# WilliamYi96/HGR-Net

Hardware: AMD Instinct MI355X
Metric: images/sec over 21K-class hierarchy, batch 512; hit@1 parity vs reference (higher is better)
Workload: dtype f16

## Files before the change

### hgr-net_amd/_lib.py

```python
from __future__ import annotations

import ctypes as C
import os
from pathlib import Path

import torch

_HERE = Path(__file__).resolve().parent
LIB_PATH = Path(os.environ.get("HGR_LIB", _HERE / "lib" / "libhgr.so"))

HGR_BF16, HGR_F16 = 0, 1
EPI_NONE, EPI_BIAS, EPI_BIAS_QUICKGELU, EPI_BIAS_RESIDUAL, EPI_BIAS_RELU, EPI_BIAS_ADD16_RELU, EPI_ACCUM, EPI_QGELU_GRAD16 = 0, 1, 2, 3, 4, 5, 6, 7

_p, _i, _l, _f = C.c_void_p, C.c_int, C.c_int64, C.c_float

SIGNATURES = {
    "hgr_gemm_nt": [_p, _l, _p, _l, _p, _l, _p, _p, _l, _i, _i, _i, _i, _i, _i, _p],
    "hgr_gemm_set_tile": [_i],
    "hgr_gemm_set_tail": [_i, _i],
    "hgr_gemm_set_persist": [_i],
    "hgr_gemm_set_ws": [_i],
    "hgr_gemm_set_p8": [_i],
    "hgr_im2col_patches": [_p, _p, _i, _i, _i, _i, _i, _p],
    "hgr_im2col_patches_ex": [_p, _p, _i, _i, _i, _i, _i, _i, _i, _p],
    "hgr_vit_assemble": [_p, _p, _p, _i, _i, _i, _p],
    "hgr_preprocess_bicubic": [_p, _p, _p, _p, _p, _p, _i, _p, _p, _i, _p, _p, C.POINTER(C.c_float), C.POINTER(C.c_float), _i, _i, _p],
    "hgr_im2col_patches_u8": [_p, _p, _i, _i, _i, _i, _i, _i, C.POINTER(C.c_float), C.POINTER(C.c_float), _i, _p],
    "hgr_vit_embed_ln": [_p, _p, _p, _p, _p, _p, _i, _i, _i, _f, _p],
    "hgr_layernorm": [_p, _p, _p, _p, _i, _i, _l, _p, _f, _i, _i, _p],
    "hgr_mha": [_p, _p, _i, _i, _i, _i, _i, _p],
    "hgr_mha_rows": [_p, _p, _i, _i, _i, _i, _i, _i, _p],
    "hgr_mha_stats": [_p, _p, _p, _i, _i, _i, _i, _i, _p],
    "hgr_text_embed": [_p, _l, _p, _p, _p, _i, _i, _i, _i, _p],
    "hgr_eot_index": [_p, _l, _p, _i, _i, _p],
    "hgr_l2norm_rows": [_p, _p, _p, _i, _i, _i, _p],
    "hgr_topk_rows": [_p, _l, _p, _i, _i, _p, _p, _i, _p],
    "hgr_level_argmax": [_p, _l, _p, _i, _p, _i, _p, _p, _i, _p],
    "hgr_eval_rows": [_p, _l, _i, _p, _p, _p, _i, _i, _p, _p, _p, _i, _i, _p, _p, _p, _i, _p],
    "hgr_conv3x3_nhwc": [_p, _p, _p, _p, _i, _i, _i, _i, _i, _i, _i, _i, _p],
    "hgr_conv3x3_pool2_nhwc": [_p, _p, _p, _p, _i, _i, _i, _i, _i, _i, _i, _p],
    "hgr_stem_conv1": [_p, _p, _p, _p, _i, _i, _i, _i, _i, _p],
    "hgr_stem_im2col": [_p, _p, _i, _i, _i, _p],
    "hgr_avgpool2_nhwc": [_p, _p, _i, _i, _i, _i, _i, _p],
    "hgr_attnpool_tokens": [_p, _p, _p, _i, _i, _i, _i, _p],
    "hgr_attnpool_attend": [_p, _p, _p, _p, _i, _i, _i, _i, _p],
    "hgr_transpose16": [_p, _l, _p, _l, _i, _i, _p],
    "hgr_transpose16_colsum": [_p, _l, _p, _l, _i, _i, _i, _p, _i, _f, _p, _p],
    "hgr_colsum": [_p, _l, _i, _i, _i, _i, _p, _i, _f, _p, _p],
    "hgr_cast16": [_p, _p, _l, _i, _p],
    "hgr_cast16_transpose": [_p, _l, _p, _l, _p, _l, _i, _i, _i, _p],
    "hgr_quickgelu16": [_p, _p, _p, _l, _i, _i, _p],
    "hgr_layernorm_bwd": [_p, _i, _p, _p, _p, _p, _p, _p, _i, _i, _l, _p, _f, _i, _p],
    "hgr_layernorm_bwd_cast": [_p, _i, _p, _p, _p, _p, _p, _p, _p, _i, _i, _l, _p, _f, _i, _p],
    "hgr_layernorm_bwd_cast_colsum": [_p, _i, _p, _p, _p, _p, _p, _p, _p, _p, _i, _i, _l, _p, _f, _i, _p],
    "hgr_layernorm_bwd_scratch_floats": [_i, _i],
    "hgr_mha_bwd": [_p, _p, _p, _p, _i, _i, _i, _i, _i, _p],
    "hgr_mha_bwd_stats": [_p, _p, _p, _p, _p, _i, _i, _i, _i, _i, _p],
    "hgr_mha_bwd_colsum": [_p, _p, _p, _p, _p, _p, _i, _i, _i, _i, _i, _p],
    "hgr_ce_rows": [_p, _l, _p, _i, _i, _f, _p, _p, _l, _p],
    "hgr_l2norm_bwd": [_p, _p, _p, _i, _i, _i, _p],
    "hgr_matmul_f32": [_p, _l, _l, _p, _l, _l, _p, _l, _i, _i, _i, _f, _i, _p],
    "hgr_embed_scatter_add": [_p, _l, _p, _p, _i, _i, _i, _i, _p],
    "hgr_rows_axpy": [_p, _l, _p, _p, _i, _i, _f, _p],
    "hgr_rows_gather": [_p, _p, _p, _i, _i, _p],
    "hgr_ctx_splice": [_p, _p, _p, _i, _i, _i, _i, _p],
    "hgr_ctx_splice_bwd": [_p, _p, _i, _i, _i, _i, _p],
    "hgr_sumsq": [_p, _l, _p, _p],
    "hgr_eval_counters": [_p, _i, _p, _i, _p, _p, _i, _p, _p, _i, _p, _i, _p],
    "hgr_eval_counters_rows": [_p, _i, _p, _p, _p, _i, _p, _p, _p, _i, _p, _i, _p],
    "hgr_eval_report_rows": [_p, _i, _p, _p, _p, _i, _p, _p, _p, _i, _p, _i, _p],
    "hgr_path_scores": [_p, _l, _p, _l, _i, _p, _p, _p, _i, _p],
    "hgr_subtree_hedge": [_p, _l, _i, _p, _p, _p, _f, _p, _i, _p, _p, _p, _l, _i, _p],
    "hgr_hedge_counters_rows": [_p, _i, _p, _p, _p, _i, _p, _i, _p],
    "hgr_set_ranks": [_p, _l, _i, _p, _p, _i, _p, _p, _p, _i, _p],
    "hgr_set_counters_rows": [_p, _p, _i, _p, _p, _i, _p, _p, _p, _i, _p, _i, _p],
    "hgr_dgp_score_rows": [_p, _l, _i, _i, _i, _f, _p, _i, _p, _i, _p, _p, _p, _p, _i, _i, _p],
    "hgr_dot_f32":[_p, _p, _l, _p, _f, _i, _p],
    "hgr_conv3x3_nhwc_plain": [_p, _p, _p, _i, _i, _i, _i, _i, _i, _i, _p],
    "hgr_gemm_nt_splitk": [_p, _l, _p, _l, _p, _l, _i, _i, _i, _i, _i, _p],
    "hgr_gemm_tn_splitk": [_p, _l, _p, _l, _p, _l, _i, _i, _i, _i, _i, _p],
    "hgr_gemm_tn_tile": [_i, _i],
    "hgr_gemm_plan_capture": [_p, _i],
    "hgr_conv3x3_wgrad_splitk": [_p, _l, _p, _p, _l, _i, _i, _i, _i, _i, _i, _i, _p],
    "hgr_relu_bwd16": [_p, _p, _p, _l, _i, _p],
    "hgr_add16": [_p, _p, _p, _l, _i, _p],
    "hgr_avgpool2_bwd_nhwc": [_p, _p, _i, _i, _i, _i, _i, _p],
    "hgr_attnpool_tokens_bwd": [_p, _p, _i, _i, _i, _i, _p],
    "hgr_im2col3x3_t": [_p, _p, _i, _i, _i, _i, _l, _i, _p],
    "hgr_bn_fold": [_p, _p, _p, _p, _p, _f, _p, _p, _i, _i, _i, _i, _i, _p],
    "hgr_bn_unfold_grad": [_p, _l, _p, _p, _p, _p, _p, _f, _p, _p, _p, _i, _i, _i, _p],
    "hgr_csr_group_aggregate": [_p, _l, _p, _p, _p, _p, _i, _p, _p, _p, _p, _i, _p, _p, _p, _p, _i, _p, _p, _l, _i, _f, _i, _p],
    "hgr_csr_group_att_grad": [_p, _l, _p, _p, _l, _p, _l, _p, _l, _p, _p, _p, _p, _i, _p, _p, _p, _i, _p, _p, _p, _i, _p, _p, _i, _f, _p],
    "hgr_dgp_loss_head": [_p, _l, _p, _p, _l, _i, _i, _p, _p, _p, _l, _i, _p],
    "hgr_dropout_counter": [_p, _l, _p, _l, _i, _i, _i, _i, _i, _p],
    "hgr_adam_l2": [_p, _p, _p, _p, _l, _f, _f, _f, _f, _f, _i, _p],
    "hgr_cnzsl_std_chain_fwd": [_p, _l, _p, _p, _p, _p, _p, _p, _l, _p, _l, _p, _i, _i, _i, _f, _f, _p],
    "hgr_cnzsl_std_chain_bwd": [_p, _l, _p, _l, _p, _l, _p, _p, _p, _l, _p, _i, _i, _f, _p],
    "hgr_bias_relu_f32": [_p, _l, _p, _p, _l, _i, _i, _p],
    "hgr_relu_bwd_colsum_f32": [_p, _l, _p, _l, _p, _l, _p, _p, _i, _i, _p],
    "hgr_gemm_nt_res_stats": [_p, _l, _p, _l, _p, _p, _l, _p, _p, _i, _i, _i, _i, _p],
    "hgr_vit_head": [_p, _p, _l, _l, _p, _p, _f, _p, _p, _i, _i, _i, _i, _p],
    "hgr_gemm_nt_res_stats_guard": [_p, _l, _p, _l, _p, _p, _l, _p, _p, _f, _p, _i, _i, _i, _i, _p],
    "hgr_gemm_nt_ln": [_p, _l, _p, _l, _p, _l, _p, _p, _p, _f, _i, _i, _i, _i, _i, _p],
    "hgr_gemm_nt_ln_mha": [_p, _l, _p, _l, _p, _p, _p, _f, _p, _l, _i, _i, _i, _i, _i, _p],
    "hgr_gemm_nt_bias_gelu_dual": [_p, _l, _p, _l, _p, _l, _p, _l, _p, _i, _i, _i, _i, _p],
    "hgr_gemm_nt_qgelu_grad_colsum": [_p, _l, _p, _l, _p, _l, _p, _l, _p, _i, _i, _i, _i, _p],
    "hgr_vit_embed_ln_stats": [_p, _p, _p, _p, _p, _p, _p, _p, _i, _i, _i, _f, _i, _p],
    "hgr_vit_patch_embed_ln_ok": [_i, _i, _i, _i, _i],
    "hgr_vit_patch_embed_ln": [_p, _p, _p, _p, _p, _p, _p, _p, _p, _i, _i, _i, _i, _f, _i, _p],
    "hgr_row_stats16": [_p, _p, _p, _p, _i, _i, _i, _p],
    "hgr_pair_rows_f32": [_p, _p, _p, _i, _i, _l, _p, _i, _p],
    "hgr_logits_eval_workspace_bytes": [_i, _i],
    "hgr_logits_eval": [_p, _p, _i, _i, _i, _p, _p, _p, _i, _p, _p, _i, _p, _i, _i, _p, _p, _p, _p, _i, _p],
    "hgr_logits_eval_tile_stage": [_p, _p, _i, _i, _i, _p, _p, _p, _i, _p, _p, _i, _p, _i, _i, _p, _p, _p, _p, _i, _p],
    "hgr_logits_eval_row_stage": [_p, _p, _i, _i, _i, _p, _p, _p, _i, _p, _p, _i, _p, _i, _i, _p, _p, _p, _p, _i, _p],
    "hgr_comm_unique_id": [_p],
    "hgr_comm_init": [_i, _i, _p],
    "hgr_comm_destroy": [],
    "hgr_comm_rank": [],
    "hgr_comm_world": [],
    "hgr_allreduce": [_p, _p, _l, _i, _i, _p],
    "hgr_allgather": [_p, _p, _l, _i, _p],
    "hgr_broadcast": [_p, _l, _i, _i, _p],
    "hgr_adamw": [_p, _p, _p, _p, _l, _f, _f, _f, _f, _f, _i, _p, _f, _f, _p],
}


class GemmLaunch(C.Structure):
    _fields_ = [(name, C.c_int32) for name in ("kernel", "variant", "epilogue", "out_f32", "act", "grid_x", "grid_y", "tiles_m", "tiles_n", "total",
                                                "nbig", "big_panels", "tiles_m_half", "group", "m_fastest", "vec_ok", "row0", "rows")]


class HgrError(RuntimeError):
    pass


_lib = None


ABI_VERSION = 5


def load() -> C.CDLL:
    global _lib
    if _lib is not None:
        return _lib
    if not LIB_PATH.is_file():
        raise HgrError(f"{LIB_PATH} not found: build it with `python -c 'import __graft_entry__ as g; g.build()'` "
                       f"or `make -C {_HERE / 'csrc'}`; there is no CPU fallback")
    lib = C.CDLL(str(LIB_PATH))
    lib.hgr_abi_version.restype = _i
    lib.hgr_last_error.restype = C.c_char_p
    for name, argtypes in SIGNATURES.items():
        fn = getattr(lib, name)
        fn.argtypes = argtypes
        fn.restype = _l if name.endswith(("_scratch_floats", "_workspace_bytes")) else _i
    if lib.hgr_abi_version() != ABI_VERSION:
        raise HgrError(f"libhgr.so ABI {lib.hgr_abi_version()} != {ABI_VERSION} (include/hgr.h): stale build, run `make -C {_HERE / 'csrc'}`")
    _lib = lib
    return lib


import threading

_tls = threading.local()


def set_muted(on: bool) -> bool:
    prev = getattr(_tls, "muted", False)
    _tls.muted = bool(on)
    return prev


def muted() -> bool:
    return getattr(_tls, "muted", False)


def call(name: str, *args) -> None:
    if getattr(_tls, "muted", False):
        return
    lib = load()
    rc = getattr(lib, name)(*args)
    if rc != 0:
        raise HgrError(f"{name} failed ({rc}): {lib.hgr_last_error().decode()}")
```

### hgr-net_amd/csrc/hgr_gemm.hip

```cpp
#include "hgr_gemm_common.h"

using namespace hgr_gemm;

int hgr_conv3x3_c32_launch(const void *x, const void *w, const float *bias, void *out, int B, int H, int W, int Cout, int Kp,
                           int dtype, int relu, void *stream, int pool, int C);

namespace {
constexpr int BM = 128, BN = 128;

HgrKnob<> k_group{"HGR_GEMM_GROUP", 0, [](int v) { return v < 0 ? 0 : v; }};
HgrKnob<> k_tail{"HGR_DUO_TAIL", 1}, k_pb{"HGR_DUO_PB", -1};
HgrKnob<double> k_half_cost{"HGR_DUO_HALF_COST", 0.55, [](double v) { return v > 0.1 ? v : 0.55; }};
HgrKnob<> k_tile{"HGR_GEMM_TILE", 0};
HgrKnob<> k_split{"HGR_GEMM_SPLIT", 1};
HgrKnob<> k_conv_direct{"HGR_CONV_DIRECT", 1}, k_conv_duo{"HGR_CONV_DUO", 1};
HgrKnob<> k_persist{"HGR_DUO_PERSIST", 1, hgr_knob_bool};
HgrKnob<> k_ws{"HGR_WS", 0, hgr_knob_bool};
HgrKnob<> k_p8{"HGR_P8", 2, [](int v) { return v >= 0 && v <= 2 ? v : 2; }};

int duo_group() { return k_group.get() ? k_group.get() : 4; }
int duo_group_for(int tiles_n) { return k_group.get() ? k_group.get() : (tiles_n <= 8 ? 1 : 4); }
int duo_dbg() {
    static const int d = hgr_lab_env("HGR_GEMM_DBG");
    return d;
// ... 266 lines not shown
GemmLaunch plan_conv3x3(const GemmArgs &a, int64_t in_pixels, bool relu, bool out16_aligned) {
    const int C = a.cC, Cout = a.N, Kp = a.K, stride = a.cStride, force = k_tile.get(), epi = relu ? HGR_EPI_BIAS_RELU : HGR_EPI_NONE;
    const int64_t t256 = (int64_t)((a.M + 255) / 256) * ((Cout + 255) / 256);
    const int waste256 = (Cout + 255) / 256 * 256 - Cout, waste128 = (Cout + 127) / 128 * 128 - Cout;
    const bool big = relu && force != 128 && Kp >= 128 && Cout >= 128 && (t256 >= 160 || force == 256) && waste256 <= waste128;
    const int64_t tduo = (int64_t)((a.M + 255) / 256) * ((Cout + 127) / 128);
    if (k_conv_duo.get() && relu && a.cUni && stride == 1 && Cout % 128 == 0 && Kp == 9 * C && tduo >= 256 && out16_aligned &&
        in_pixels * C * 2 < (1ll << 31) && (int64_t)Cout * Kp * 2 < (1ll << 32) && force == 0)
        return plan_duo(a, 5, HGR_EPI_BIAS_RELU, false);
    if (big) return plan_tiles(HGR_KERNEL_256, 1, HGR_EPI_BIAS_RELU, false, a.M, Cout, 256, 256);
    if (Cout <= 64 && a.M >= 1024) return plan_tiles(HGR_KERNEL_128, V128_CONV_TALL, epi, false, a.M, 1, 256, 1);
    return plan_tiles(HGR_KERNEL_128, V128_CONV, epi, false, a.M, Cout, BM, BN);
}

int conv3x3_launch(const void *x, const void *w, const float *bias, void *out,
                   int B, int H, int W, int C, int Cout, int stride, int Kp, int dtype, bool relu, void *stream) {
    CaptureScope capture;
    HGR_REQUIRE(x && w && out && (bias || !relu), "hgr_conv3x3_nhwc: null operand");
    HGR_REQUIRE(B >= 1 && H >= 1 && W >= 1 && Cout >= 1 && (stride == 1 || stride == 2), "hgr_conv3x3_nhwc: bad geometry B=%d H=%d W=%d Cout=%d stride=%d", B, H, W, Cout, stride);
    HGR_REQUIRE(C >= 8 && C % 8 == 0 && C <= 16384, "hgr_conv3x3_nhwc: C=%d must be a multiple of 8 in [8, 16384]", C);
    HGR_REQUIRE(Kp >= 9 * C && Kp % BK == 0, "hgr_conv3x3_nhwc: Kp=%d must be >= 9*C and a multiple of %d", Kp, BK);
    HGR_REQUIRE(hgr_aligned(x, 16) && hgr_aligned(w, 16) && hgr_aligned(out, 8) && (!bias || hgr_aligned(bias, 16)) && Cout % 4 == 0, "hgr_conv3x3_nhwc: misaligned operand / Cout %% 4 != 0");
    HGR_REQUIRE(dtype == HGR_BF16 || dtype == HGR_F16, "hgr_conv3x3_nhwc: bad dtype %d", dtype);
    if (const int direct = conv_direct_channels(C, Cout, stride, Kp, (int64_t)B * H * W, hgr_aligned(out, 16))) {
        if (cap_out) { *cap_out = hgr_gemm_launch{HGR_KERNEL_CONV_DIRECT, direct, relu ? HGR_EPI_BIAS_RELU : HGR_EPI_NONE, 0, relu}; return HGR_OK; }
        return hgr_conv3x3_c32_launch(x, w, bias, out, B, H, W, Cout, Kp, dtype, relu ? 1 : 0, stream, 0, direct);
    }
    const int Ho = (H + 2 - 3) / stride + 1, Wo = (W + 2 - 3) / stride + 1;
    const int64_t M64 = (int64_t)B * Ho * Wo;
    HGR_REQUIRE(M64 < (1ll << 31), "hgr_conv3x3_nhwc: too many output pixels");
    GemmArgs a = gemm_args(x, 0, w, Kp, out, Cout, (int)M64, Cout, Kp, true, 0);
    a.bias = bias; a.m_fastest = 0;
    a.cH = H; a.cW = W; a.cC = C; a.cStride = stride; a.cHo = Ho; a.cWo = Wo;
    a.cMagic = (unsigned)(((1ull << 32) + (unsigned)C - 1) / (unsigned)C);
    a.cUni = (C % 64 == 0) ? 1 : 0;
    const GemmLaunch L = plan_conv3x3(a, (int64_t)B * H * W, relu, hgr_aligned(out, 16));
    return gemm_run("hgr_conv3x3_nhwc", a, &L, 1, dtype, stream);
}
}

extern "C" int hgr_conv3x3_nhwc(const void *x, const void *w, const float *bias, void *out,
                                int B, int H, int W, int C, int Cout, int stride, int Kp, int dtype, void *stream) {
    return conv3x3_launch(x, w, bias, out, B, H, W, C, Cout, stride, Kp, dtype, true, stream);
}

extern "C" int hgr_conv3x3_nhwc_plain(const void *x, const void *w, void *out, int B, int H, int W, int C, int Cout, int Kp,
                                      int dtype, void *stream) {
    return conv3x3_launch(x, w, nullptr, out, B, H, W, C, Cout, 1, Kp, dtype, false, stream);
}

extern "C" int hgr_gemm_nt_splitk(const void *A, int64_t lda, const void *W, int64_t ldw, float *partial, int64_t ldc,
                                  int M, int N, int K, int kc, int dtype, void *stream) {
    CaptureScope capture;
    HGR_REQUIRE(A && W && partial, "hgr_gemm_nt_splitk: null operand");
    HGR_REQUIRE(M >= 1 && N >= 1 && K >= BK && K % BK == 0 && kc >= BK && kc % BK == 0, "hgr_gemm_nt_splitk: bad shape M=%d N=%d K=%d kc=%d", M, N, K, kc);
    HGR_REQUIRE(lda >= K && ldw >= K && lda % 8 == 0 && ldw % 8 == 0 && hgr_aligned(A, 16) && hgr_aligned(W, 16), "hgr_gemm_nt_splitk: operands must be 16-byte aligned with leading dimensions %% 8 == 0");
    HGR_REQUIRE(ldc >= N && ldc % 4 == 0 && hgr_aligned(partial, 16), "hgr_gemm_nt_splitk: partial must be 16-byte aligned, ldc %% 4 == 0");
    HGR_REQUIRE(dtype == HGR_BF16 || dtype == HGR_F16, "hgr_gemm_nt_splitk: bad dtype %d", dtype);
    const int S = (K + kc - 1) / kc;
    HGR_REQUIRE(S <= 65535, "hgr_gemm_nt_splitk: %d splits exceed the grid limit", S);
    GemmArgs a = gemm_args(A, lda, W, ldw, partial, ldc, M, N, K, true, 0);
    a.m_fastest = 0; a.kc = kc; a.csplit = (int64_t)M * ldc;
    const bool big = k_tile.get() != 128 && M >= 256 && N >= 256 && kc >= 128 && (K - (S - 1) * kc) >= 128;
    const GemmLaunch L = big ? plan_tiles(HGR_KERNEL_256, 0, HGR_EPI_NONE, true, M, N, 256, 256, (unsigned)S)
                             : plan_tiles(HGR_KERNEL_128, V128_PLAIN, HGR_EPI_NONE, true, M, N, BM, BN, (unsigned)S);
    return gemm_run("hgr_gemm_nt_splitk", a, &L, 1, dtype, stream);
}

namespace {
int ln_common_checks(const char *who, const void *A, int64_t lda, const void *W, int64_t ldw, int M, int N, int K, int dtype) {
    HGR_REQUIRE(A && W, "%s: null operand", who);
    HGR_REQUIRE(M >= 1 && N >= 128 && N % 128 == 0 && K >= 128 && K % 64 == 0, "%s: bad shape M=%d N=%d K=%d (N %% 128 == 0, K %% 64 == 0, K >= 128)", who, M, N, K);
    HGR_REQUIRE(lda >= K && ldw >= K && lda % 8 == 0 && ldw % 8 == 0 && hgr_aligned(A, 16) && hgr_aligned(W, 16), "%s: operands must be 16-byte aligned with leading dimensions %% 8 == 0", who);
    HGR_REQUIRE((int64_t)M * lda * 2 < (1ll << 32) && (int64_t)N * ldw * 2 < (1ll << 32) && N < (1 << 20), "%s: operands beyond 4 GB / N >= 2^20", who);
    HGR_REQUIRE(dtype == HGR_BF16 || dtype == HGR_F16, "%s: bad dtype %d", who, dtype);
    return HGR_OK;
}
}

extern "C" int hgr_gemm_nt_res_stats(const void *A, int64_t lda, const void *W, int64_t ldw, void *xh, void *xl, int64_t ldx,
                                     const float *bias, float *stats, int M, int N, int K, int dtype, void *stream) {
    return hgr_gemm_nt_res_stats_guard(A, lda, W, ldw, xh, xl, ldx, bias, stats, 0.f, nullptr, M, N, K, dtype, stream);
}

extern "C" int hgr_gemm_nt_res_stats_guard(const void *A, int64_t lda, const void *W, int64_t ldw, void *xh, void *xl, int64_t ldx,
                                           const float *bias, float *stats, float guard_sumsq, uint32_t *flag,
                                           int M, int N, int K, int dtype, void *stream) {
    CaptureScope capture;
    if (int rc = ln_common_checks("hgr_gemm_nt_res_stats", A, lda, W, ldw, M, N, K, dtype)) return rc;
    HGR_REQUIRE(!flag || (guard_sumsq > 0.f && hgr_aligned(flag, 4)), "hgr_gemm_nt_res_stats_guard: flag needs guard_sumsq > 0 and 4-byte alignment");
    HGR_REQUIRE(xh && xl && bias && stats, "hgr_gemm_nt_res_stats: null xh / xl / bias / stats");
    HGR_REQUIRE(ldx >= N && ldx % 8 == 0 && ldx < (1 << 23) && hgr_aligned(xh, 16) && hgr_aligned(xl, 16), "hgr_gemm_nt_res_stats: xh / xl must be 16-byte aligned, ldx %% 8 == 0, ldx < 2^23");
    HGR_REQUIRE(hgr_aligned(bias, 16) && hgr_aligned(stats, 8), "hgr_gemm_nt_res_stats: bias must be 16-byte, stats 8-byte aligned");
    GemmArgs a = gemm_args(A, lda, W, ldw, nullptr, 0, M, N, K, true, duo_dbg());
    a.bias = bias;
    a.ln_stats = stats; a.ln_slots = N / 64; a.ln_xh = xh; a.ln_xl = xl; a.ln_ldx = ldx;
    a.ln_flag = flag; a.ln_guard = guard_sumsq;
    const GemmLaunch L = k_ws.get() && k_tile.get() == 0 && ws_covers(M, N, K, WS_LNP) ? plan_ws(M, N, WS_LNP, HGR_EPI_BIAS_RESIDUAL, 0)
                                                                                        : plan_duo(a, 1, HGR_EPI_BIAS_RESIDUAL, true);
    return gemm_run("hgr_gemm_nt_res_stats", a, &L, 1, dtype, stream);
}

extern "C" int hgr_gemm_nt_ln(const void *X16, int64_t ldx, const void *Wfold, int64_t ldw, void *C, int64_t ldc,
                              const float *ln_s, const float *ln_c, const float *stats, float eps,
                              int M, int N, int K, int dtype, int act, void *stream) {
    CaptureScope capture;
    if (int rc = ln_common_checks("hgr_gemm_nt_ln", X16, ldx, Wfold, ldw, M, N, K, dtype)) return rc;
    HGR_REQUIRE(C && ln_s && ln_c && stats, "hgr_gemm_nt_ln: null C / ln_s / ln_c / stats");
    HGR_REQUIRE(K % 128 == 0, "hgr_gemm_nt_ln: the row width K=%d must be a multiple of 128 (two 64-column statistic slots per 16-byte load)", K);
    HGR_REQUIRE(ldc >= N && ldc % 8 == 0 && ldc < (1 << 23) && hgr_aligned(C, 16), "hgr_gemm_nt_ln: C must be 16-byte aligned with ldc %% 8 == 0, ldc < 2^23");
    HGR_REQUIRE(hgr_aligned(ln_s, 16) && hgr_aligned(ln_c, 16) && hgr_aligned(stats, 16), "hgr_gemm_nt_ln: ln_s / ln_c / stats must be 16-byte aligned");
    HGR_REQUIRE(act == 0 || act == 1, "hgr_gemm_nt_ln: act must be 0 (none) or 1 (QuickGELU), got %d", act);
    GemmArgs a = gemm_args(X16, ldx, Wfold, ldw, C, ldc, M, N, K, true, duo_dbg());
    a.ln_stats = const_cast<float *>(stats); a.ln_slots = K / 64; a.ln_eps = eps; a.ln_s = ln_s; a.ln_c = ln_c;
    const int epi = act ? HGR_EPI_BIAS_QUICKGELU : HGR_EPI_BIAS;
    const GemmLaunch L = k_tile.get() == 0 && p8_wanted(M, N, K)                           ? plan_p8(M, N, act)
                         : k_ws.get() && k_tile.get() == 0 && ws_covers(M, N, K, WS_LNC) ? plan_ws(M, N, WS_LNC, epi, act)
                                                                                          : plan_duo(a, 2, epi, false);
    return gemm_run("hgr_gemm_nt_ln", a, &L, 1, dtype, stream);
}

extern "C" int hgr_gemm_nt_bias_gelu_dual(const void *A, int64_t lda, const void *W, int64_t ldw, void *pre, int64_t ldpre, void *post, int64_t ldpost,
                                          const float *bias, int M, int N, int K, int dtype, void *stream) {
    CaptureScope capture;
    if (int rc = ln_common_checks("hgr_gemm_nt_bias_gelu_dual", A, lda, W, ldw, M, N, K, dtype)) return rc;
    HGR_REQUIRE(pre && post && bias, "hgr_gemm_nt_bias_gelu_dual: null pre / post / bias");
    HGR_REQUIRE(ldpre >= N && ldpost >= N && ldpre % 8 == 0 && ldpost % 8 == 0 && ldpre < (1 << 23) && ldpost < (1 << 23) && hgr_aligned(pre, 16) && hgr_aligned(post, 16) && hgr_aligned(bias, 16),
                "hgr_gemm_nt_bias_gelu_dual: pre / post / bias must be 16-byte aligned, leading dimensions >= N, %% 8 == 0, < 2^23");
    GemmArgs a = gemm_args(A, lda, W, ldw, pre, ldpre, M, N, K, true, duo_dbg());
    a.bias = bias; a.ln_xh = post; a.ln_ldx = ldpost;
    const GemmLaunch L = plan_duo(a, 4, HGR_EPI_BIAS, false);
    return gemm_run("hgr_gemm_nt_bias_gelu_dual", a, &L, 1, dtype, stream);
}

extern "C" int hgr_gemm_nt_qgelu_grad_colsum(const void *A, int64_t lda, const void *W, int64_t ldw, void *C, int64_t ldc, const void *pre, int64_t ldpre,
                                             float *colsum_part, int M, int N, int K, int dtype, void *stream) {
    CaptureScope capture;
    if (int rc = ln_common_checks("hgr_gemm_nt_qgelu_grad_colsum", A, lda, W, ldw, M, N, K, dtype)) return rc;
    HGR_REQUIRE(C && pre && colsum_part, "hgr_gemm_nt_qgelu_grad_colsum: null C / pre / colsum_part");
    HGR_REQUIRE(ldc >= N && ldpre >= N && ldc % 8 == 0 && ldpre % 8 == 0 && ldc < (1 << 20) && ldpre < (1 << 20) && hgr_aligned(C, 16) && hgr_aligned(pre, 16) && hgr_aligned(colsum_part, 16),
                "hgr_gemm_nt_qgelu_grad_colsum: C / pre / colsum_part must be 16-byte aligned, leading dimensions >= N, %% 8 == 0, < 2^20");
    GemmArgs a = gemm_args(A, lda, W, ldw, C, ldc, M, N, K, true, duo_dbg());
    a.res = (const float *)pre; a.ldr = ldpre;
    a.colsum = colsum_part; a.colsum_units = (M + 63) / 64;
    const GemmLaunch L = plan_duo(a, 0, HGR_EPI_QGELU_GRAD16, false);
    return gemm_run("hgr_gemm_nt_qgelu_grad_colsum", a, &L, 1, dtype, stream);
}

#define HGR_LE_PARAMS const void *feat16, const void *zsl_perm16, int rows, int D, int n_perm, const int32_t *tpos_perm, const int32_t *epos_perm, \
    const int32_t *level_first, int n_levels, const int32_t *filler_pos, const int32_t *train_cols, int n_train, const int32_t *test_cols, int n_test, int k, \
    int32_t *out_level, int32_t *out_top1, int32_t *out_topk, void *workspace, int dtype, void *stream
#define HGR_LE_ARGS feat16, zsl_perm16, rows, D, n_perm, tpos_perm, epos_perm, level_first, n_levels, filler_pos, train_cols, n_train, test_cols, n_test, k, \
    out_level, out_top1, out_topk, workspace, dtype, stream
static int logits_eval_stages(int stages, HGR_LE_PARAMS);
extern "C" int hgr_logits_eval(HGR_LE_PARAMS) { return logits_eval_stages(3, HGR_LE_ARGS); }
extern "C" int hgr_logits_eval_tile_stage(HGR_LE_PARAMS) { return logits_eval_stages(1, HGR_LE_ARGS); }
extern "C" int hgr_logits_eval_row_stage(HGR_LE_PARAMS) { return logits_eval_stages(2, HGR_LE_ARGS); }

int hgr_logits_eval_rows_launch(const void *feat, const void *zslp, int D, int S, const unsigned long long *keys, const float *tmax,
                                const int *gp1, const float *gm2, const int32_t *level_first, int n_levels, const int32_t *filler_pos, const int32_t *train_cols, int n_train,
                                const int32_t *epos, const int32_t *test_cols, int n_test, int k, int32_t *out_level, int32_t *out_top1,
                                int32_t *out_topk, int rows, int dtype, void *stream);

extern "C" int64_t hgr_logits_eval_workspace_bytes(int rows, int n_perm) {
    if (rows < 1 || n_perm < 96 || n_perm % 96) return -1;
    return (int64_t)rows * (n_perm / 32) * 32;
}

static int logits_eval_stages(int stages, const void *feat16, const void *zsl_perm16, int rows, int D, int n_perm,
                               const int32_t *tpos_perm, const int32_t *epos_perm, const int32_t *level_first,
                               int n_levels, const int32_t *filler_pos, const int32_t *train_cols, int n_train,
                               const int32_t *test_cols, int n_test, int k,
                               int32_t *out_level, int32_t *out_top1, int32_t *out_topk, void *workspace, int dtype, void *stream) {
    HGR_REQUIRE(feat16 && zsl_perm16 && tpos_perm && epos_perm && level_first && filler_pos && train_cols && out_level && workspace, "hgr_logits_eval: null operand");
    HGR_REQUIRE(rows >= 1 && D >= 128 && D % 128 == 0 && D <= 1024, "hgr_logits_eval: rows=%d D=%d unsupported (D %% 128 == 0, D <= 1024)", rows, D);
    HGR_REQUIRE(n_perm >= 96 && n_perm % 96 == 0 && n_perm / 32 <= 1024, "hgr_logits_eval: n_perm=%d must be a multiple of 96 and <= 32768 (32-column level-aligned slices, 96-column slabs)", n_perm);
    HGR_REQUIRE(n_levels >= 1 && n_levels <= 32 && n_train >= 1, "hgr_logits_eval: bad sizes (n_levels <= 32)");
    HGR_REQUIRE(k == 0 || (out_topk && test_cols && k >= 1 && k <= 32 && n_test >= k), "hgr_logits_eval: bad top-k arguments");
    HGR_REQUIRE(hgr_aligned(feat16, 16) && hgr_aligned(zsl_perm16, 16) && hgr_aligned(tpos_perm, 16) && hgr_aligned(epos_perm, 16) && hgr_aligned(workspace, 16), "hgr_logits_eval: operands must be 16-byte aligned");
    HGR_REQUIRE(dtype == HGR_BF16 || dtype == HGR_F16, "hgr_logits_eval: bad dtype %d", dtype);
    HGR_REQUIRE((int64_t)rows * D * 2 < (1ll << 32) && (int64_t)n_perm * D * 2 < (1ll << 32), "hgr_logits_eval: operands beyond 4 GB");
    const int S = n_perm / 32;
    SlabArgs a;
    a.A = (const char *)feat16; a.lda = D; a.W = (const char *)zsl_perm16; a.ldw = D; a.M = rows; a.K = D; a.Np = n_perm;
    a.tpos = tpos_perm; a.epos = epos_perm; a.S = S;
    { static const int d = hgr_lab_env("HGR_LS_DBG"); a.dbg = d; }
    a.ev_key = (unsigned long long *)workspace;
    a.ev_tmax = (float *)((char *)workspace + (size_t)rows * S * 8);
    a.ev_p1 = (int *)((char *)workspace + (size_t)rows * S * 16);
    a.ev_m2 = (float *)((char *)workspace + (size_t)rows * S * 24);
    if (stages & 1) launch_logits_slab(a, dtype, (hipStream_t)stream);
    HGR_CHECK_LAUNCH("hgr_logits_eval (tile stage)");
    if (!(stages & 2)) return HGR_OK;
    return hgr_logits_eval_rows_launch(feat16, zsl_perm16, D, S, a.ev_key, a.ev_tmax, a.ev_p1, a.ev_m2, level_first, n_levels, filler_pos, train_cols, n_train,
                                       epos_perm, test_cols, n_test, k, out_level, out_top1, out_topk, rows, dtype, stream);
}
```

### hgr-net_amd/csrc/hgr_gemm_common.h

```cpp
#pragma once
#include "hgr_common.h"
#include <stdlib.h>
#include <type_traits>

namespace hgr_gemm {

constexpr int BK = 64;

struct GemmArgs {
    const char *A = nullptr; int64_t lda = 0;
    const char *W = nullptr; int64_t ldw = 0;
    void *C = nullptr; int64_t ldc = 0;
    const float *bias = nullptr;
    const float *res = nullptr; int64_t ldr = 0;
    int M = 0, N = 0, K = 0;
    int tiles_m = 0, tiles_n = 0;
    int m_fastest = 0;
    int vec_ok = 0;
    int dbg = 0;
    int cH = 0, cW = 0, cC = 0, cStride = 0, cHo = 0, cWo = 0;
    unsigned cMagic = 0;
    int cUni = 0;
    int kc = 0; int64_t csplit = 0;
    float *ln_stats = nullptr; int ln_slots = 0; float ln_eps = 0.f;
// ... 91 lines not shown
    return o;
}

__host__ __device__ constexpr bool epi_has_bias(int epi) { return epi != HGR_EPI_NONE && epi != HGR_EPI_ACCUM && epi != HGR_EPI_QGELU_GRAD16; }
__host__ __device__ constexpr bool epi_has_idn16(int epi) { return epi == HGR_EPI_BIAS_ADD16_RELU || epi == HGR_EPI_QGELU_GRAD16; }

template <int DT, int EPI, bool OUT32>
__device__ __forceinline__ void store_quad(const GemmArgs &p, f32x4 v, int m, int n) {
    typedef typename T16<DT>::elem E;
    if (n + 3 < p.N && p.vec_ok) {
        if (epi_has_bias(EPI)) v += *(const f32x4 *)(p.bias + n);
        if (EPI == HGR_EPI_ACCUM) v += *(const f32x4 *)((const float *)p.C + (int64_t)m * p.ldc + n);
        const f32x4 v0 = v;
        f32x4 gq = (f32x4){0.f, 0.f, 0.f, 0.f};
        if (EPI == HGR_EPI_BIAS_QUICKGELU) {
#pragma unroll
            for (int e = 0; e < 4; ++e) v[e] = quick_gelu(v[e]);
        }
        if (EPI == HGR_EPI_BIAS_RESIDUAL) v += *(const f32x4 *)(p.res + (int64_t)m * p.ldr + n);
        if (epi_has_idn16(EPI)) {
            const typename T16<DT>::vec4 idn = *(const typename T16<DT>::vec4 *)((const E *)(const void *)p.res + (int64_t)m * p.ldr + n);
#pragma unroll
            for (int e = 0; e < 4; ++e) {
                if (EPI == HGR_EPI_QGELU_GRAD16) { gq[e] = quick_gelu_grad((float)idn[e]); v[e] = v[e] * gq[e]; }
                else v[e] = v[e] + (float)idn[e];
            }
        }
        if (EPI == HGR_EPI_BIAS_RELU || EPI == HGR_EPI_BIAS_ADD16_RELU) {
#pragma unroll
            for (int e = 0; e < 4; ++e) v[e] = fmaxf(v[e], 0.f);
        }
        if (OUT32) *(f32x4 *)((float *)p.C + (int64_t)m * p.ldc + n) = v;
        else if (EPI == HGR_EPI_BIAS_QUICKGELU || EPI == HGR_EPI_QGELU_GRAD16) {
            typename T16<DT>::vec4 o;
#pragma unroll
            for (int e = 0; e < 4; ++e) o[e] = EPI == HGR_EPI_BIAS_QUICKGELU ? quick_gelu16<DT>(v0[e]) : mul16<DT>(v0[e], gq[e]);
            *(typename T16<DT>::vec4 *)((E *)p.C + (int64_t)m * p.ldc + n) = o;
        } else *(typename T16<DT>::vec4 *)((E *)p.C + (int64_t)m * p.ldc + n) = cvt4<DT>(v[0], v[1], v[2], v[3]);
        return;
    }
    for (int e = 0; e < 4 && n + e < p.N; ++e) {
        float x = v[e];
        if (epi_has_bias(EPI)) x += p.bias[n + e];
        if (EPI == HGR_EPI_ACCUM) x += ((const float *)p.C)[(int64_t)m * p.ldc + n + e];
        const float x0 = x;
        float gx = 0.f;
        if (EPI == HGR_EPI_BIAS_QUICKGELU) x = quick_gelu(x);
        if (EPI == HGR_EPI_BIAS_RESIDUAL) x += p.res[(int64_t)m * p.ldr + n + e];
        if (EPI == HGR_EPI_BIAS_ADD16_RELU) x += (float)((const E *)(const void *)p.res)[(int64_t)m * p.ldr + n + e];
        if (EPI == HGR_EPI_QGELU_GRAD16) { gx = quick_gelu_grad((float)((const E *)(const void *)p.res)[(int64_t)m * p.ldr + n + e]); x *= gx; }
        if (EPI == HGR_EPI_BIAS_RELU || EPI == HGR_EPI_BIAS_ADD16_RELU) x = fmaxf(x, 0.f);
        if (OUT32) ((float *)p.C)[(int64_t)m * p.ldc + n + e] = x;
        else if (EPI == HGR_EPI_BIAS_QUICKGELU) ((E *)p.C)[(int64_t)m * p.ldc + n + e] = quick_gelu16<DT>(x0);
        else if (EPI == HGR_EPI_QGELU_GRAD16) ((E *)p.C)[(int64_t)m * p.ldc + n + e] = mul16<DT>(x0, gx);
        else ((E *)p.C)[(int64_t)m * p.ldc + n + e] = (E)x;
    }
}

template <int DT, int EPI>
__device__ __forceinline__ f32x4 load_addend(const GemmArgs &p, int m, int n) {
    typedef typename T16<DT>::elem E;
    if (EPI == HGR_EPI_ACCUM) return *(const f32x4 *)((const float *)p.C + (int64_t)m * p.ldc + n);
    if (EPI == HGR_EPI_BIAS_RESIDUAL) return *(const f32x4 *)(p.res + (int64_t)m * p.ldr + n);
    if (epi_has_idn16(EPI)) {
        const typename T16<DT>::vec4 idn = *(const typename T16<DT>::vec4 *)((const E *)(const void *)p.res + (int64_t)m * p.ldr + n);
        return (f32x4){(float)idn[0], (float)idn[1], (float)idn[2], (float)idn[3]};
    }
    return (f32x4){0.f, 0.f, 0.f, 0.f};
}

template <int DT, int EPI, bool OUT32>
__device__ __forceinline__ void store_quad_full(const GemmArgs &p, f32x4 v, f32x4 bq, f32x4 addend, int m, int n) {
    typedef typename T16<DT>::elem E;
    if (epi_has_bias(EPI)) v += bq;
    if (!OUT32 && (EPI == HGR_EPI_BIAS_QUICKGELU || EPI == HGR_EPI_QGELU_GRAD16)) {
        typename T16<DT>::vec4 o;
#pragma unroll
        for (int e = 0; e < 4; ++e) o[e] = EPI == HGR_EPI_BIAS_QUICKGELU ? quick_gelu16<DT>(v[e]) : mul16<DT>(v[e], quick_gelu_grad(addend[e]));
        *(typename T16<DT>::vec4 *)((E *)p.C + (int64_t)m * p.ldc + n) = o;
        return;
    }
    if (EPI == HGR_EPI_BIAS_QUICKGELU) {
#pragma unroll
        for (int e = 0; e < 4; ++e) v[e] = quick_gelu(v[e]);
    }
    if (EPI == HGR_EPI_ACCUM || EPI == HGR_EPI_BIAS_RESIDUAL || EPI == HGR_EPI_BIAS_ADD16_RELU) v += addend;
    if (EPI == HGR_EPI_QGELU_GRAD16) {
#pragma unroll
        for (int e = 0; e < 4; ++e) v[e] *= quick_gelu_grad(addend[e]);
    }
    if (EPI == HGR_EPI_BIAS_RELU || EPI == HGR_EPI_BIAS_ADD16_RELU) {
#pragma unroll
        for (int e = 0; e < 4; ++e) v[e] = fmaxf(v[e], 0.f);
    }
    if (OUT32) *(f32x4 *)((float *)p.C + (int64_t)m * p.ldc + n) = v;
    else *(typename T16<DT>::vec4 *)((E *)p.C + (int64_t)m * p.ldc + n) = cvt4<DT>(v[0], v[1], v[2], v[3]);
}


__device__ __forceinline__ __amdgpu_buffer_rsrc_t dma_rsrc(const void *base) {
    return __builtin_amdgcn_make_buffer_rsrc(const_cast<void *>(base), 0, (int)0xFFFFFFFFu, 0x00020000);
}
__device__ __forceinline__ void dma16(__amdgpu_buffer_rsrc_t rsrc, const char *base, unsigned voff, int soff, char *lds_dst) {
#if defined(HGR_DMA_GLOBAL) && HGR_DMA_GLOBAL
    __builtin_amdgcn_global_load_lds((const AS1 void *)(base + soff + voff), (AS3 void *)lds_dst, 16, 0, 0);
#else
    __builtin_amdgcn_raw_ptr_buffer_load_lds(rsrc, (AS3 void *)lds_dst, 16, (int)voff, soff, 0, 0);
#endif
}

#define HGR_RWAIT(N) do { __builtin_amdgcn_sched_barrier(0); \
    asm volatile("s_waitcnt vmcnt(" #N ") lgkmcnt(0)\n\ts_barrier" ::: "memory"); __builtin_amdgcn_sched_barrier(0); } while (0)
#define HGR_RBAR() do { __builtin_amdgcn_sched_barrier(0); \
    asm volatile("s_waitcnt lgkmcnt(0)\n\ts_barrier" ::: "memory"); __builtin_amdgcn_sched_barrier(0); } while (0)
#define HGR_MBAR() do { __builtin_amdgcn_sched_barrier(0); \
    asm volatile("s_barrier" ::: "memory"); __builtin_amdgcn_sched_barrier(0); } while (0)


template <int NR, int NW, int NV, int M_, int NM = 16>
__device__ __forceinline__ void mfma16_interleave_step() {
    if constexpr (M_ < NM) {
        __builtin_amdgcn_sched_group_barrier(0x008, 1, 0);
        constexpr int DR = (M_ + 1) * NR / NM - M_ * NR / NM, DW = (M_ + 1) * NW / NM - M_ * NW / NM, DV = (M_ + 1) * NV / NM - M_ * NV / NM;
        if constexpr (DR > 0) __builtin_amdgcn_sched_group_barrier(0x100, DR, 0);
        if constexpr (DW > 0) __builtin_amdgcn_sched_group_barrier(0x200, DW, 0);
        if constexpr (DV > 0) __builtin_amdgcn_sched_group_barrier(0x020, DV, 0);
        mfma16_interleave_step<NR, NW, NV, M_ + 1, NM>();
    }
}
template <int NR, int NW, int NV>
__device__ __forceinline__ void mfma16_interleave() { mfma16_interleave_step<NR, NW, NV, 0>(); }
template <int NR, int NW, int NV>
__device__ __forceinline__ void mfma8_interleave() { mfma16_interleave_step<NR, NW, NV, 0, 8>(); }

enum { V128_PLAIN = 0, V128_TALL = 1, V128_CONV = 2, V128_CONV_TALL = 3 };
void launch_128(const GemmArgs &a, int dtype, int epi, bool out32, int variant, dim3 grid, hipStream_t s);
void launch_256(const GemmArgs &a, int dtype, int epi, bool out32, bool conv, dim3 grid, hipStream_t s);
void launch_duo(const GemmArgs &a, int dtype, int epi, bool out32, int ln, dim3 grid, hipStream_t s);
enum { WS_PLAIN = 0, WS_LNC = 1, WS_LNP = 2 };
bool ws_covers(int M, int N, int K, int mode);
int ws_cus();
void launch_ws(const GemmArgs &a, int dtype, int mode, int act, bool hasb, dim3 grid, hipStream_t s);
bool p8_covers(int M, int N, int K);
void launch_p8(const GemmArgs &a, int dtype, int act, dim3 grid, hipStream_t s);

struct SlabArgs {
    const char *A = nullptr; int64_t lda = 0;
    const char *W = nullptr; int64_t ldw = 0;
    int M = 0, K = 0, Np = 0;
    const int *tpos = nullptr, *epos = nullptr;
    unsigned long long *ev_key = nullptr;
    float *ev_tmax = nullptr, *ev_m2 = nullptr; int *ev_p1 = nullptr;
    int S = 0;
    int dbg = 0;
};
void launch_logits_slab(const SlabArgs &a, int dtype, hipStream_t s);

}
```

### hgr-net_amd/csrc/hgr_logits_slab.hip

```cpp
#include "hgr_gemm_common.h"

namespace hgr_gemm {

namespace {
constexpr int LS_NT = 512;
constexpr int LS_PA0 = 0, LS_PA1 = 32768, LS_PW = 65536, LS_STAGE = 81920, LS_LDS = 2 * LS_STAGE;

template <int DT>
__global__ __launch_bounds__(LS_NT) void logits_slab(SlabArgs p) {
    typedef typename T16<DT>::vec8 vec8;
    __shared__ __attribute__((aligned(1024))) char smem[LS_LDS];

    const int tid = threadIdx.x;
    const int lane = tid & 63;
    const int wave = __builtin_amdgcn_readfirstlane(tid >> 6);
    const int pg = wave >> 2;
    const int r = lane & 15, g = lane >> 4;
    const int n0 = blockIdx.x * 96, m0 = blockIdx.y * 512;

    unsigned oA0[4], oA1[4], oW[2];
#pragma unroll
    for (int i = 0; i < 4; ++i) {
        const int id = (i * 8 + wave) * 64 + lane;
        const int pr = id >> 3, c = (id & 7) ^ (pr & 7);
        const int tr = (pr >> 5) * 64 + (pr & 31);
        oA0[i] = (unsigned)(((int64_t)min(m0 + tr, p.M - 1) * p.lda + c * 8) * 2);
        oA1[i] = (unsigned)(((int64_t)min(m0 + tr + 32, p.M - 1) * p.lda + c * 8) * 2);
        if (i < 2) oW[i] = (unsigned)(((int64_t)(n0 + min(pr, 95)) * p.ldw + c * 8) * 2);
    }
    unsigned tw[6], ta;
    {
        const int spr = p.K >> 5;
        const int nw = 96 * spr;
#pragma unroll
        for (int u = 0; u < 6; ++u) {
            const int id = min(tid + u * LS_NT, nw - 1);
            tw[u] = HGR_LAB_ON(p.dbg & 16) ? 0u : *(const unsigned *)(p.W + ((int64_t)(n0 + id / spr) * p.ldw) * 2 + (id % spr) * 64);
        }
        const int rows_here = min(512, p.M - m0), na = rows_here * spr;
        const int id = min((int)(blockIdx.x >> 3) * LS_NT + tid, na - 1);
        ta = *(const unsigned *)(p.A + ((int64_t)(m0 + id / spr) * p.lda) * 2 + (id % spr) * 64);
    }
    char *const ldsw = smem + wave * 1024;
    const __amdgpu_buffer_rsrc_t rA = dma_rsrc(p.A), rW = dma_rsrc(p.W);
    auto issueA = [&](const unsigned (&off)[4], int piece, int t) {
        if (HGR_LAB_ON(p.dbg & 2)) return;
        char *dst = ldsw + (t & 1) * LS_STAGE + piece;
#pragma unroll
        for (int i = 0; i < 4; ++i) dma16(rA, p.A, off[i], t * 128, dst + i * 8192);
    };
    auto issueW = [&](int t) {
        if (HGR_LAB_ON(p.dbg & 4)) return;
        char *dst = ldsw + (t & 1) * LS_STAGE + LS_PW;
#pragma unroll
        for (int i = 0; i < 2; ++i) dma16(rW, p.W, oW[i], t * 128, dst + i * 8192);
    };

    f32x4 acc[4][6];
#pragma unroll
    for (int i = 0; i < 4; ++i)
#pragma unroll
        for (int j = 0; j < 6; ++j) acc[i][j] = (f32x4){0.f, 0.f, 0.f, 0.f};

    const int nk = p.K / 64;
    const int offA = (wave * 32 + r) * 128;
    const int offW = r * 128;
    const int sw0 = ((0 + g) ^ (r & 7)) * 16, sw1 = ((4 + g) ^ (r & 7)) * 16;
    vec8 wf[6][2], af[2][2];

    issueA(oA0, LS_PA0, 0); issueW(0);
    issueA(oA1, LS_PA1, 0);
    issueA(oA0, LS_PA0, 1); issueW(1);
    HGR_RWAIT(10);
    if (pg) HGR_MBAR();

    auto ktile = [&](int t, auto mode_tag) {
        constexpr int MODE = decltype(mode_tag)::value;
        const char *st = smem + (t & 1) * LS_STAGE;
        if (MODE <= 1) issueA(oA1, LS_PA1, t + 1);
#pragma unroll
        for (int j = 0; j < 6; ++j) {
            wf[j][0] = *(const vec8 *)(st + LS_PW + offW + j * 2048 + sw0);
            wf[j][1] = *(const vec8 *)(st + LS_PW + offW + j * 2048 + sw1);
        }
#pragma unroll
        for (int i = 0; i < 2; ++i) {
            af[i][0] = *(const vec8 *)(st + LS_PA0 + offA + i * 2048 + sw0);
            af[i][1] = *(const vec8 *)(st + LS_PA0 + offA + i * 2048 + sw1);
        }
        if (MODE <= 1) HGR_RWAIT(10); else HGR_RWAIT(0);
        __builtin_amdgcn_s_setprio(1);
#pragma unroll
        for (int kk = 0; kk < 2; ++kk)
#pragma unroll
            for (int i = 0; i < 2; ++i)
#pragma unroll
                for (int j = 0; j < 6; ++j) if (!HGR_LAB_ON(p.dbg & 1)) acc[i][j] = T16<DT>::mfma16(wf[j][kk], af[i][kk], acc[i][j]);
        __builtin_amdgcn_s_setprio(0);
        HGR_MBAR();
        if (MODE == 0) { issueA(oA0, LS_PA0, t + 2); issueW(t + 2); }
#pragma unroll
        for (int i = 0; i < 2; ++i) {
            af[i][0] = *(const vec8 *)(st + LS_PA1 + offA + i * 2048 + sw0);
            af[i][1] = *(const vec8 *)(st + LS_PA1 + offA + i * 2048 + sw1);
        }
        if (MODE == 0) HGR_RWAIT(10); else if (MODE == 1) HGR_RWAIT(4); else HGR_RBAR();
        __builtin_amdgcn_s_setprio(1);
#pragma unroll
        for (int kk = 0; kk < 2; ++kk)
#pragma unroll
            for (int i = 0; i < 2; ++i)
#pragma unroll
                for (int j = 0; j < 6; ++j) if (!HGR_LAB_ON(p.dbg & 1)) acc[2 + i][j] = T16<DT>::mfma16(wf[j][kk], af[i][kk], acc[2 + i][j]);
        __builtin_amdgcn_s_setprio(0);
        HGR_MBAR();
    };
    for (int t = 0; t < nk - 2; ++t) ktile(t, std::integral_constant<int, 0>());
    ktile(nk - 2, std::integral_constant<int, 1>());
    ktile(nk - 1, std::integral_constant<int, 2>());
    if (!pg) HGR_MBAR();

    if (HGR_LAB_ON(p.dbg & 8)) { if (acc[0][0][0] == 123.456f && acc[3][5][3] == 1.f) p.ev_key[0] = 1ull; return; }
    int tp[6][4], ep[6][4];
#pragma unroll
    for (int j = 0; j < 6; ++j) {
        const int n = n0 + j * 16 + g * 4;
        const int4 t4 = *(const int4 *)(p.tpos + n), e4 = *(const int4 *)(p.epos + n);
        tp[j][0] = t4.x; tp[j][1] = t4.y; tp[j][2] = t4.z; tp[j][3] = t4.w;
        ep[j][0] = e4.x; ep[j][1] = e4.y; ep[j][2] = e4.z; ep[j][3] = e4.w;
    }
    char *const rec = (char *)p.ev_key + (int64_t)blockIdx.x * p.M * 96 + g * 24;
#define LS_SWAP16(x) __builtin_amdgcn_permlane16_swap((unsigned)(x), (unsigned)(x), false, false)
#define LS_SWAP32(x) __builtin_amdgcn_permlane32_swap((unsigned)(x), (unsigned)(x), false, false)
    auto xmaxf = [&](float v) {
        auto a = LS_SWAP16(__float_as_uint(v));
        v = fmaxf(__uint_as_float(a[0]), __uint_as_float(a[1]));
        auto b = LS_SWAP32(__float_as_uint(v));
        return fmaxf(__uint_as_float(b[0]), __uint_as_float(b[1]));
    };
    auto xmini = [&](int v) {
        auto a = LS_SWAP16(v);
        v = min((int)a[0], (int)a[1]);
        auto b = LS_SWAP32(v);
        return min((int)b[0], (int)b[1]);
    };
#pragma unroll
    for (int i = 0; i < 4; ++i) {
        const int m = m0 + wave * 64 + i * 16 + r;
#pragma unroll
        for (int s = 0; s < 3; ++s) {
            float m1[2], m2[2];
            int p1[2];
            float tv[2][4];
            float V = -INFINITY;
#pragma unroll
            for (int jj = 0; jj < 2; ++jj)
#pragma unroll
                for (int e = 0; e < 4; ++e) {
                    tv[jj][e] = tp[2 * s + jj][e] >= 0 ? acc[i][2 * s + jj][e] + 0.0f : -INFINITY;
                    V = fmaxf(V, tv[jj][e]);
                }
            V = xmaxf(V);
            int P = 0x7fffffff;
#pragma unroll
            for (int jj = 0; jj < 2; ++jj)
#pragma unroll
                for (int e = 0; e < 4; ++e) P = min(P, (tp[2 * s + jj][e] >= 0 && tv[jj][e] == V) ? tp[2 * s + jj][e] : 0x7fffffff);
            P = xmini(P);
            const unsigned long long vkey = key_of(V, P);
            const unsigned long long key = P == 0x7fffffff ? 0ull : vkey;
#pragma unroll
            for (int jj = 0; jj < 2; ++jj) {
                const int j = 2 * s + jj;
                float x[4];
#pragma unroll
                for (int e = 0; e < 4; ++e) x[e] = ep[j][e] >= 0 ? acc[i][j][e] + 0.0f : -INFINITY;
                const float hi01 = fmaxf(x[0], x[1]), lo01 = fminf(x[0], x[1]), hi23 = fmaxf(x[2], x[3]), lo23 = fminf(x[2], x[3]);
                float t1 = fmaxf(hi01, hi23);
                float t2 = fmaxf(fminf(hi01, hi23), fmaxf(lo01, lo23));
                int q1 = x[0] == t1 ? ep[j][0] : x[1] == t1 ? ep[j][1] : x[2] == t1 ? ep[j][2] : ep[j][3];
                {
                    auto a1 = LS_SWAP16(__float_as_uint(t1)); auto a2 = LS_SWAP16(__float_as_uint(t2)); auto ap = LS_SWAP16(q1);
                    const float e1 = __uint_as_float(a1[0]), o1 = __uint_as_float(a1[1]);
                    t2 = fmaxf(fminf(e1, o1), fmaxf(__uint_as_float(a2[0]), __uint_as_float(a2[1])));
                    q1 = o1 > e1 ? (int)ap[1] : (int)ap[0];
                    t1 = fmaxf(e1, o1);
                }
                {
                    auto a1 = LS_SWAP32(__float_as_uint(t1)); auto a2 = LS_SWAP32(__float_as_uint(t2)); auto ap = LS_SWAP32(q1);
                    const float e1 = __uint_as_float(a1[0]), o1 = __uint_as_float(a1[1]);
                    t2 = fmaxf(fminf(e1, o1), fmaxf(__uint_as_float(a2[0]), __uint_as_float(a2[1])));
                    q1 = o1 > e1 ? (int)ap[1] : (int)ap[0];
                    t1 = fmaxf(e1, o1);
                }
                m1[jj] = t1; m2[jj] = t2; p1[jj] = q1;
            }
            if (m < p.M || ((tw[0] ^ tw[1] ^ tw[2]) + (tw[3] ^ tw[4] ^ tw[5]) + ta == 0x9E3779B9u && m == 0x7fffffff)) {
                const unsigned long long v8 = g == 0 ? key
                    : g == 1 ? ((unsigned long long)__float_as_uint(m1[1]) << 32) | __float_as_uint(m1[0])
                    : g == 2 ? ((unsigned long long)(unsigned)p1[1] << 32) | (unsigned)p1[0]
                             : ((unsigned long long)__float_as_uint(m2[1]) << 32) | __float_as_uint(m2[0]);
                *(unsigned long long *)(rec + (int64_t)m * 96 + s * 8) = v8;
            }
        }
    }
#undef LS_SWAP16
#undef LS_SWAP32
}
}

void launch_logits_slab(const SlabArgs &a, int dtype, hipStream_t s) {
    const dim3 grid((unsigned)(a.Np / 96), (unsigned)((a.M + 511) / 512)), block(LS_NT);
    if (dtype == HGR_BF16) hipLaunchKernelGGL((logits_slab<HGR_BF16>), grid, block, 0, s, a);
    else hipLaunchKernelGGL((logits_slab<HGR_F16>), grid, block, 0, s, a);
}

}
```

### hgr-net_amd/csrc/hgr_select.hip

```cpp
#include "hgr_common.h"
#include <math.h>

namespace {

struct Best { float v; int p; };

__device__ __forceinline__ bool better(float v, int p, float bv, int bp) { return v > bv || (v == bv && p < bp); }

__device__ __forceinline__ Best best_of_key(unsigned long long m) {
    Best b = {-INFINITY, 0x7fffffff};
    if (m) key_decode(m, b.v, b.p);
    return b;
}

__device__ __forceinline__ Best wave_best(Best b) {
#pragma unroll
    for (int o = 32; o > 0; o >>= 1) {
        const float ov = __shfl_xor(b.v, o);
        const int op = __shfl_xor(b.p, o);
        if (better(ov, op, b.v, b.p)) { b.v = ov; b.p = op; }
    }
    return b;
}

template <int NW>
__device__ __forceinline__ Best block_best(Best b, float *s_v, int *s_p, int tid) {
    const Best w = wave_best(b);
    __syncthreads();
    if ((tid & 63) == 0) { s_v[tid >> 6] = w.v; s_p[tid >> 6] = w.p; }
    __syncthreads();
    Best r = {s_v[0], s_p[0]};
    for (int i = 1; i < NW; ++i)
        if (better(s_v[i], s_p[i], r.v, r.p)) { r.v = s_v[i]; r.p = s_p[i]; }
    return r;
}

__device__ __forceinline__ int level_winner(Best b, int fo, int n_train) {
    const bool has_c = b.p < n_train, has_f = fo >= 0;
    if (has_c && (!has_f || b.v > -1.0f || (b.v == -1.0f && b.p < fo))) return b.p;
    return has_f ? fo : b.p;
}

__device__ __forceinline__ void slice_threshold(const float *s_mv, const int *s_mp, int k, int tid, float &s_t, int &s_tp) {
    if (tid < 256) {
        const float mv = s_mv[tid]; const int mp = s_mp[tid];
        int rank = 0, nonempty = 0;
        for (int j = 0; j < 256; ++j) { rank += better(s_mv[j], s_mp[j], mv, mp) ? 1 : 0; nonempty += s_mp[j] != 0x7fffffff ? 1 : 0; }
        if (nonempty < k) { if (tid == 0) { s_t = -INFINITY; s_tp = 0x7fffffff; } }
        else if (rank == k - 1) { s_t = mv; s_tp = mp; }
    }
}

template <int NT, typename F>
__device__ __forceinline__ void rank_and_emit(const float *s_cv, const int *s_cp, int cnt, int k, int tid, F emit) {
    for (int c = tid; c < cnt; c += NT) {
        const float v = s_cv[c]; const int p = s_cp[c];
        int rk = 0;
        for (int j = 0; j < cnt; ++j) rk += better(s_cv[j], s_cp[j], v, p) ? 1 : 0;
        if (rk < k) emit(rk, v, p);
    }
}

template <int NT>
__device__ __forceinline__ void topk_rounds(const float *lr, int n_nodes, const int32_t *test_pos, const int32_t *test_cols, int n_test, int k,
                                            int32_t *out, float *s_v, int *s_p, int tid) {
    Best last = {INFINITY, -1};
    for (int j = 0; j < k; ++j) {
        Best b = {-INFINITY, 0x7fffffff};
        for (int c = tid; c < n_nodes; c += NT) {
            const int te = test_pos[c];
            if (te < 0) continue;
            const float v = lr[c] + 0.0f;
            if (better(last.v, last.p, v, te) && better(v, te, b.v, b.p)) { b.v = v; b.p = te; }
        }
        b = block_best<NT / 64>(b, s_v, s_p, tid);
        if (tid == 0) out[j] = b.p < n_test ? test_cols[b.p] : -1;
        last = b;
        __syncthreads();
    }
}

constexpr int TOPK_CAND = 1024;

__global__ __launch_bounds__(256) void topk_rows(const float *__restrict__ logits, int64_t ld, const int32_t *__restrict__ cols,
                                                 int n_cols, int k, int32_t *__restrict__ out_idx, float *__restrict__ out_val) {
    extern __shared__ __attribute__((aligned(16))) char dyn[];
    float *vals = (float *)dyn;
    __shared__ float s_mv[256];
    __shared__ int s_mp[256];
    __shared__ float s_cv[TOPK_CAND];
    __shared__ int s_cp[TOPK_CAND];
    __shared__ float s_t;
    __shared__ int s_tp, s_cnt;
    const int tid = threadIdx.x;
    const int row = blockIdx.x;
    const float *lr = logits + (int64_t)row * ld;
    Best mine = {-INFINITY, 0x7fffffff};
    for (int p = tid; p < n_cols; p += 256) {
        const float v = lr[cols ? cols[p] : p];
        vals[p] = v;
        if (v > mine.v) { mine.v = v; mine.p = p; }
    }
    s_mv[tid] = mine.v; s_mp[tid] = mine.p;
    if (tid == 0) s_cnt = 0;
    __syncthreads();
    int rank = 0;
    for (int j = 0; j < 256; ++j) rank += better(s_mv[j], s_mp[j], mine.v, mine.p) ? 1 : 0;
    const int kth = min(k, n_cols) - 1;
    if (rank == min(kth, min(n_cols, 256) - 1)) { s_t = mine.v; s_tp = mine.p; }
    __syncthreads();
    const float t = s_t; const int tp = s_tp;
    if (!better(t, tp, mine.v, mine.p)) {
        for (int p = tid; p < n_cols; p += 256) {
            const float v = vals[p];
            if (!better(t, tp, v, p)) {
                const int slot = atomicAdd(&s_cnt, 1);
                if (slot < TOPK_CAND) { s_cv[slot] = v; s_cp[slot] = p; }
            }
        }
    }
    __syncthreads();
    const int cnt = s_cnt;
    if (cnt <= TOPK_CAND) {
        rank_and_emit<256>(s_cv, s_cp, cnt, k, tid, [&](int rk, float v, int p) {
            out_idx[(int64_t)row * k + rk] = cols ? cols[p] : p;
            if (out_val) out_val[(int64_t)row * k + rk] = v;
        });
        return;
    }
    auto scan = [&]() {
        Best b = {-INFINITY, 0x7fffffff};
        for (int p = tid; p < n_cols; p += 256) {
            const float v = vals[p];
            if (v > b.v) { b.v = v; b.p = p; }
        }
        return b;
    };
    for (int j = 0; j < k; ++j) {
        const Best b = block_best<4>(mine, s_mv, s_mp, tid);
        if (tid == 0) {
            const bool ok = b.p < n_cols;
            out_idx[(int64_t)row * k + j] = ok ? (cols ? cols[b.p] : b.p) : -1;
            if (out_val) out_val[(int64_t)row * k + j] = b.v;
            if (ok) vals[b.p] = -INFINITY;
        }
        __syncthreads();
        if (mine.p == b.p) mine = scan();
    }
}

template <int NLV>
__global__ __launch_bounds__(256) void level_argmax(const float *__restrict__ logits, int64_t ld, const int32_t *__restrict__ cols,
                                                    int n_cols, const int32_t *__restrict__ depth, int n_levels, int32_t *__restrict__ out, int32_t *__restrict__ out_top1) {
    __shared__ float s_v[4][NLV];
    __shared__ float s_bv[NLV];
    __shared__ int s_bp[NLV];
    __shared__ int s_p[4][NLV];
    __shared__ int s_fd[4];
    const int tid = threadIdx.x, lane = tid & 63, wave = tid >> 6;
    const int row = blockIdx.x;
    const float *lr = logits + (int64_t)row * ld;
    float bv[NLV];
    int bp[NLV];
#pragma unroll
    for (int l = 0; l < NLV; ++l) { bv[l] = -INFINITY; bp[l] = 0x7fffffff; }
    const int lvl0 = depth[cols ? cols[0] : 0];
    int fd = 0x7fffffff;
    for (int p0 = tid; p0 < n_cols; p0 += 4 * 256) {
        int c4[4], lv4[4];
        float v4[4];
#pragma unroll
        for (int u = 0; u < 4; ++u) { const int p = min(p0 + u * 256, n_cols - 1); c4[u] = cols ? cols[p] : p; }
#pragma unroll
        for (int u = 0; u < 4; ++u) { lv4[u] = depth[c4[u]]; v4[u] = lr[c4[u]]; }
#pragma unroll
        for (int u = 0; u < 4; ++u) {
            const int p = p0 + u * 256;
            if (p >= n_cols) break;
            const int lv = lv4[u];
            const float v = v4[u];
            if (lv != lvl0 && p < fd) fd = p;
#pragma unroll
            for (int l = 0; l < NLV; ++l)
                if (lv == l && v > bv[l]) { bv[l] = v; bp[l] = p; }
        }
    }
#pragma unroll
    for (int o = 32; o > 0; o >>= 1) fd = min(fd, __shfl_xor(fd, o));
#pragma unroll
    for (int l = 0; l < NLV; ++l) {
        Best b = {bv[l], bp[l]};
        b = wave_best(b);
        if (lane == 0) { s_v[wave][l] = b.v; s_p[wave][l] = b.p; }
    }
    if (lane == 0) s_fd[wave] = fd;
    __syncthreads();
    if (tid < n_levels) {
        const int l = tid;
        Best b = {s_v[0][l], s_p[0][l]};
#pragma unroll
        for (int i = 1; i < 4; ++i)
            if (better(s_v[i][l], s_p[i][l], b.v, b.p)) { b.v = s_v[i][l]; b.p = s_p[i][l]; }
        const int fdd = min(min(s_fd[0], s_fd[1]), min(s_fd[2], s_fd[3]));
        const int fo = (l != lvl0) ? 0 : fdd;
        const int win = level_winner(b, fo < n_cols ? fo : -1, n_cols);
        out[(int64_t)row * n_levels + l] = cols ? cols[win] : win;
        s_bv[l] = b.v; s_bp[l] = b.p;
    }
    if (out_top1) {
        __syncthreads();
        if (tid == 0) {
            Best b = {-INFINITY, 0x7fffffff};
            for (int l = 0; l < n_levels; ++l)
                if (better(s_bv[l], s_bp[l], b.v, b.p)) { b.v = s_bv[l]; b.p = s_bp[l]; }
            out_top1[row] = b.p < n_cols ? (cols ? cols[b.p] : b.p) : -1;
        }
    }
}

constexpr int EV_NT = 1024;
constexpr int EV_NW = EV_NT / 64;
constexpr int EV_NLV = 32;

__global__ __launch_bounds__(EV_NT) void eval_rows(const float *__restrict__ logits, int64_t ld, int n_nodes, const unsigned char *__restrict__ lvl8,
                                                 const int32_t *__restrict__ train_pos, const int32_t *__restrict__ train_cols, int n_train, int n_levels,
                                                 const int32_t *__restrict__ filler_pos, const int32_t *__restrict__ test_pos, const int32_t *__restrict__ test_cols,
                                                 int n_test, int k, int32_t *__restrict__ out_level, int32_t *__restrict__ out_top1, int32_t *__restrict__ out_topk) {
    __shared__ float s_lv[EV_NW][EV_NLV];
    __shared__ int s_lp[EV_NW][EV_NLV];
    __shared__ float s_v[EV_NW];
    __shared__ int s_p[EV_NW];
    __shared__ float s_mv[256];
// ... 26 lines not shown
#pragma unroll
    for (int l = 0; l < EV_NLV; ++l) {
        Best b = {bv[l], bp[l]};
        b = wave_best(b);
        if (lane == 0) { s_lv[wave][l] = b.v; s_lp[wave][l] = b.p; }
    }
    {
        Best gmx = mine;
#pragma unroll
        for (int o = 1; o <= 2; o <<= 1) {
            const float ov = __shfl_xor(gmx.v, o);
            const int op = __shfl_xor(gmx.p, o);
            if (better(ov, op, gmx.v, gmx.p)) { gmx.v = ov; gmx.p = op; }
        }
        if ((tid & 3) == 0) { s_mv[tid >> 2] = gmx.v; s_mp[tid >> 2] = gmx.p; }
    }
    __syncthreads();
    if (wave == 0) {
        const int l = lane;
        Best b = {-INFINITY, 0x7fffffff};
        if (l < n_levels) {
            b = Best{s_lv[0][l], s_lp[0][l]};
            for (int i = 1; i < EV_NW; ++i)
                if (better(s_lv[i][l], s_lp[i][l], b.v, b.p)) { b.v = s_lv[i][l]; b.p = s_lp[i][l]; }
            out_level[(int64_t)r * n_levels + l] = train_cols[level_winner(b, filler_pos[l], n_train)];
        }
        const Best top = wave_best(b);
        if (lane == 0 && out_top1) out_top1[r] = top.p < n_train ? train_cols[top.p] : -1;
    }
    if (k <= 0) return;
    slice_threshold(s_mv, s_mp, k, tid, s_t, s_tp);
    __syncthreads();
    const float t = s_t; const int tp0 = s_tp;
    for (int c = tid; c < n_nodes; c += EV_NT) {
        const int te = test_pos[c];
        if (te < 0) continue;
        const float v = lr[c] + 0.0f;
        if (!better(t, tp0, v, te)) {
            const int slot = atomicAdd(&s_cnt, 1);
            if (slot < TOPK_CAND) { s_cv[slot] = v; s_cp[slot] = te; }
        }
    }
    __syncthreads();
    const int cnt = s_cnt;
    int32_t *out = out_topk + (int64_t)r * k;
    if (cnt <= TOPK_CAND) rank_and_emit<EV_NT>(s_cv, s_cp, cnt, k, tid, [&](int rk, float, int p) { out[rk] = test_cols[p]; });
    else topk_rounds<EV_NT>(lr, n_nodes, test_pos, test_cols, n_test, k, out, s_v, s_p, tid);
}

constexpr int EL_NT = 512, EL_NW = EL_NT / 64, EL_NLV = 16;
constexpr int EL_U = 8;

__global__ __launch_bounds__(EL_NT) void eval_rows_lds(const float *__restrict__ logits, int64_t ld, int n_nodes, const unsigned char *__restrict__ lvl8,
                                                 const int32_t *__restrict__ train_pos, const int32_t *__restrict__ train_cols, int n_train, int n_levels,
                                                 const int32_t *__restrict__ filler_pos, const int32_t *__restrict__ test_pos, const int32_t *__restrict__ test_cols,
                                                 int n_test, int k, int32_t *__restrict__ out_level, int32_t *__restrict__ out_top1, int32_t *__restrict__ out_topk) {
    __shared__ unsigned long long acc[EL_NLV][EL_NT];
    __shared__ unsigned long long s_key[EL_NLV];
    __shared__ float s_v[EL_NW];
    __shared__ int s_p[EL_NW];
    __shared__ float s_mv[256];
    __shared__ int s_mp[256];
    __shared__ float s_cv[TOPK_CAND];
    __shared__ int s_cp[TOPK_CAND];
    __shared__ float s_t;
    __shared__ int s_tp, s_cnt;
    const int tid = threadIdx.x, lane = tid & 63, wave = tid >> 6;
    const int r = blockIdx.x;
    const float *lr = logits + (int64_t)r * ld;
    if (tid == 0) s_cnt = 0;
#pragma unroll
    for (int l = 0; l < EL_NLV; ++l) acc[l][tid] = 0ull;
    Best mine = {-INFINITY, 0x7fffffff};
    for (int c0 = tid; c0 < n_nodes; c0 += EL_U * EL_NT) {
        float v4[EL_U]; int tp4[EL_U], lv4[EL_U], te4[EL_U];
#pragma unroll
        for (int u4 = 0; u4 < EL_U; ++u4) {
            const int c = min(c0 + u4 * EL_NT, n_nodes - 1);
            v4[u4] = lr[c]; tp4[u4] = train_pos[c]; lv4[u4] = lvl8[c]; te4[u4] = k > 0 ? test_pos[c] : -1;
        }
#pragma unroll
        for (int u4 = 0; u4 < EL_U; ++u4) {
            if (c0 + u4 * EL_NT >= n_nodes) break;
            const float v = v4[u4] + 0.0f;
            const int tp = tp4[u4];
            if (tp >= 0 && lv4[u4] < EL_NLV) {
                const unsigned long long key = key_of(v, tp);
                unsigned long long *slot = &acc[lv4[u4]][tid];
                if (key > *slot) *slot = key;
            }
            const int te = te4[u4];
            if (te >= 0 && better(v, te, mine.v, mine.p)) { mine.v = v; mine.p = te; }
        }
    }
    {
        Best gmx = mine;
#pragma unroll
        for (int o = 1; o <= 1; o <<= 1) {
            const float ov = __shfl_xor(gmx.v, o);
            const int op = __shfl_xor(gmx.p, o);
            if (better(ov, op, gmx.v, gmx.p)) { gmx.v = ov; gmx.p = op; }
        }
        if ((tid & 1) == 0) { s_mv[tid >> 1] = gmx.v; s_mp[tid >> 1] = gmx.p; }
    }
    __syncthreads();
    for (int l = wave; l < EL_NLV; l += EL_NW) {
        unsigned long long m = 0ull;
#pragma unroll
        for (int i = 0; i < EL_NT / 64; ++i) { const unsigned long long x = acc[l][lane + 64 * i]; m = x > m ? x : m; }
        m = wave_max_u64(m);
        if (lane == 0) s_key[l] = m;
    }
    __syncthreads();
    if (wave == 0) {
        const int l = lane;
        Best b = {-INFINITY, 0x7fffffff};
        if (l < n_levels) {
            b = best_of_key(l < EL_NLV ? s_key[l] : 0ull);
            out_level[(int64_t)r * n_levels + l] = train_cols[level_winner(b, filler_pos[l], n_train)];
        }
        const Best top = wave_best(b);
        if (lane == 0 && out_top1) out_top1[r] = top.p < n_train ? train_cols[top.p] : -1;
    }
    if (k <= 0) return;
    slice_threshold(s_mv, s_mp, k, tid, s_t, s_tp);
    __syncthreads();
    const float t = s_t; const int tp0 = s_tp;
    for (int c0 = tid; c0 < n_nodes; c0 += EL_U * EL_NT) {
        float v4[EL_U]; int te4[EL_U];
#pragma unroll
        for (int u4 = 0; u4 < EL_U; ++u4) {
            const int c = min(c0 + u4 * EL_NT, n_nodes - 1);
            v4[u4] = lr[c]; te4[u4] = test_pos[c];
        }
#pragma unroll
        for (int u4 = 0; u4 < EL_U; ++u4) {
            if (c0 + u4 * EL_NT >= n_nodes) break;
            const int te = te4[u4];
            const float v = v4[u4] + 0.0f;
            if (te >= 0 && !better(t, tp0, v, te)) {
                const int slot = atomicAdd(&s_cnt, 1);
                if (slot < TOPK_CAND) { s_cv[slot] = v; s_cp[slot] = te; }
            }
        }
    }
    __syncthreads();
    const int cnt = s_cnt;
    int32_t *out = out_topk + (int64_t)r * k;
    if (cnt <= TOPK_CAND) rank_and_emit<EL_NT>(s_cv, s_cp, cnt, k, tid, [&](int rk, float, int p) { out[rk] = test_cols[p]; });
    else topk_rounds<EL_NT>(lr, n_nodes, test_pos, test_cols, n_test, k, out, s_v, s_p, tid);
}


constexpr int LE_NT = 512, LE_NW = LE_NT / 64, LE_MAXS = 1024, LE_CAP = 2048, LE_GPS = 2;

template <int DT>
__global__ __launch_bounds__(LE_NT, 4) void logits_eval_rows(const void *__restrict__ feat, const void *__restrict__ zslp, int D, int S,
                                                        const unsigned long long *__restrict__ keys, const float *__restrict__ gmax,
                                                        const int *__restrict__ gp1, const float *__restrict__ gm2,
                                                        const int32_t *__restrict__ level_first, int n_levels, const int32_t *__restrict__ filler_pos,
                                                        const int32_t *__restrict__ train_cols, int n_train, const int32_t *__restrict__ epos,
                                                        const int32_t *__restrict__ test_cols, int n_test, int k,
                                                        int32_t *__restrict__ out_level, int32_t *__restrict__ out_top1, int32_t *__restrict__ out_topk, int dbg, int rows) {
    typedef typename T16<DT>::vec8 vec8;
    typedef typename T16<DT>::elem E;
    __shared__ unsigned long long s_lkey[32];
    __shared__ unsigned long long s_keys[LE_MAXS];
    __shared__ __attribute__((aligned(16))) float s_gm[LE_MAXS * LE_GPS];
    __shared__ __attribute__((aligned(16))) float s_m2[LE_MAXS * LE_GPS];
    __shared__ __attribute__((aligned(16))) int s_p1[LE_MAXS * LE_GPS];
    __shared__ float s_tm[LE_MAXS];
    __shared__ short s_cand[LE_MAXS * LE_GPS];
    __shared__ __attribute__((aligned(16))) E s_feat[1024];
    __shared__ float s_cv[LE_CAP];
    __shared__ int s_cp[LE_CAP];
    __shared__ float s_t;
    __shared__ int s_ncand, s_cnt, s_nonempty;
    __shared__ float s_bv[LE_NW];
    __shared__ int s_bp[LE_NW];
    const int tid = threadIdx.x, lane = tid & 63, wave = tid >> 6;
    const int row = blockIdx.x;
    if (tid < 32) s_lkey[tid] = 0ull;
    if (tid == 0) { s_ncand = 0; s_cnt = 0; s_nonempty = 0; s_t = -INFINITY; }
    {
        const int s0 = tid, s1 = tid + LE_NT;
        const int c0s = min(s0, S - 1), c1s = min(s1, S - 1);
        const char *r0 = (const char *)keys + ((int64_t)(c0s / 3) * rows + row) * 96 + (c0s % 3) * 8;
        const char *r1 = (const char *)keys + ((int64_t)(c1s / 3) * rows + row) * 96 + (c1s % 3) * 8;
        const unsigned long long k0 = *(const unsigned long long *)r0, k1 = *(const unsigned long long *)r1;
        const float2 a0 = *(const float2 *)(r0 + 24), a1 = *(const float2 *)(r1 + 24);
        const int2 c0 = *(const int2 *)(r0 + 48), c1 = *(const int2 *)(r1 + 48);
        const float2 b0 = *(const float2 *)(r0 + 72), b1 = *(const float2 *)(r1 + 72);
        u32x4 fv = (u32x4){0u, 0u, 0u, 0u};
        if (tid < (D >> 3)) fv = ((const u32x4 *)((const E *)feat + (int64_t)row * D))[tid];
        int mine = 0;
        if (s0 < S) {
            s_keys[s0] = k0; *(float2 *)(s_gm + s0 * LE_GPS) = a0; *(float2 *)(s_m2 + s0 * LE_GPS) = b0; *(int2 *)(s_p1 + s0 * LE_GPS) = c0;
            const float t = fmaxf(a0.x, a0.y);
            s_tm[s0] = t;
            mine += t > -INFINITY ? 1 : 0;
        }
        if (s1 < S) {
            s_keys[s1] = k1; *(float2 *)(s_gm + s1 * LE_GPS) = a1; *(float2 *)(s_m2 + s1 * LE_GPS) = b1; *(int2 *)(s_p1 + s1 * LE_GPS) = c1;
            const float t = fmaxf(a1.x, a1.y);
            s_tm[s1] = t;
            mine += t > -INFINITY ? 1 : 0;
        }
        if (tid < (D >> 3)) ((u32x4 *)s_feat)[tid] = fv;
#pragma unroll
        for (int o = 32; o > 0; o >>= 1) mine += __shfl_xor(mine, o);
        if (lane == 0 && mine) atomicAdd(&s_nonempty, mine);
    }
    __syncthreads();
    const bool want_k = k > 0 && !HGR_LAB_ON(dbg == 1);
    if (wave == 0 && want_k && s_nonempty >= k) {
        unsigned kv[LE_MAXS / 64];
        const int nreg = (S + 63) >> 6;
        unsigned best = 0;
#pragma unroll
        for (int i = 0; i < LE_MAXS / 64; ++i) {
            const int s = i * 64 + lane;
            kv[i] = orderable(s < S ? s_tm[s] : -INFINITY);
            best = max(best, kv[i]);
        }
        const unsigned ninf = 0x007FFFFFu;
        const int lanes_live = __popcll(__ballot(best > ninf));
        unsigned x = 0;
        if (lanes_live >= k) {
            int rk = 0;
            for (int j = 0; j < 64; ++j) {
                const unsigned o = (unsigned)__builtin_amdgcn_readlane((int)best, j);
                rk += (o > best || (o == best && j < lane)) ? 1 : 0;
            }
            const unsigned long long pick = __ballot(rk == k - 1);
            x = (unsigned)__builtin_amdgcn_readlane((int)best, (int)__builtin_ctzll(pick));
        } else {
            for (int bit = 31; bit >= 0; --bit) {
                const unsigned c = x | (1u << bit);
                int cntc = 0;
#pragma unroll
                for (int i = 0; i < LE_MAXS / 64; ++i)
                    if (i < nreg) cntc += __popcll(__ballot(kv[i] >= c));
                if (cntc >= k) x = c;
            }
        }
        if (lane == 0) s_t = unorderable(x);
    } else if (wave > 0 || !want_k || s_nonempty < k) {
        const int w0 = (want_k && s_nonempty >= k) ? 1 : 0, nw = LE_NW - w0;
        for (int l = wave - w0; l < n_levels; l += nw) {
            unsigned long long m = 0ull;
            for (int s = level_first[l] + lane; s < level_first[l + 1]; s += 64) { const unsigned long long x = s_keys[s]; m = x > m ? x : m; }
            m = wave_max_u64(m);
            if (lane == 0) s_lkey[l] = m;
        }
    }
    __syncthreads();
    if (wave == LE_NW - 1) {
        const int l = lane;
        Best b = {-INFINITY, 0x7fffffff};
        if (l < n_levels) {
            b = best_of_key(l < 32 ? s_lkey[l] : 0ull);
            out_level[(int64_t)row * n_levels + l] = train_cols[level_winner(b, filler_pos[l], n_train)];
        }
        const Best top = wave_best(b);
        if (lane == 0 && out_top1) out_top1[row] = top.p < n_train ? train_cols[top.p] : -1;
    }
    if (!want_k) return;
    if (HGR_LAB_ON(dbg == 2)) return;
    const float t = s_t;
    for (int q = tid; q < S * LE_GPS; q += LE_NT) {
        const float m1 = s_gm[q];
        if (m1 > -INFINITY && m1 >= t) {
            if (s_m2[q] >= t) s_cand[atomicAdd(&s_ncand, 1)] = (short)q;
            else {
                const int slot = atomicAdd(&s_cnt, 1);
                if (slot < LE_CAP) { s_cv[slot] = m1; s_cp[slot] = s_p1[q]; }
            }
        }
    }
    __syncthreads();
    int ncand = s_ncand;
    if (HGR_LAB_ON(dbg == 3)) return;
    const int r16 = lane & 15, g = lane >> 4;
    const int ks = D >> 5;
    auto scan = [&](auto visit) {
        for (int ci = wave * 2; ci < ncand; ci += 2 * LE_NW) {
            const int q0 = s_cand[ci], q1 = s_cand[min(ci + 1, ncand - 1)];
            const E *w0 = (const E *)zslp + ((int64_t)q0 * 16 + r16) * D + g * 8;
            const E *w1 = (const E *)zslp + ((int64_t)q1 * 16 + r16) * D + g * 8;
            f32x4 a0 = (f32x4){0.f, 0.f, 0.f, 0.f}, a1 = a0;
            for (int kk = 0; kk < ks; kk += 8) {
                vec8 f0[8], f1[8];
#pragma unroll
                for (int u = 0; u < 8; ++u) {
                    const int kq = min(kk + u, ks - 1);
                    f0[u] = *(const vec8 *)(w0 + kq * 32); f1[u] = *(const vec8 *)(w1 + kq * 32);
                }
#pragma unroll
                for (int u = 0; u < 8; ++u) {
                    if (kk + u < ks) {
                        const vec8 xf = *(const vec8 *)(s_feat + (kk + u) * 32 + g * 8);
                        a0 = T16<DT>::mfma16(f0[u], xf, a0);
                        a1 = T16<DT>::mfma16(f1[u], xf, a1);
                    }
                }
            }
            float v0 = r16 == 0 ? a0[0] : r16 == 1 ? a0[1] : r16 == 2 ? a0[2] : a0[3];
            float v1 = r16 == 0 ? a1[0] : r16 == 1 ? a1[1] : r16 == 2 ? a1[2] : a1[3];
            v0 += 0.0f; v1 += 0.0f;
            if (r16 < 4) {
                const int te0 = epos[q0 * 16 + g * 4 + r16];
                if (te0 >= 0) visit(v0, te0);
                if (ci + 1 < ncand) {
                    const int te1 = epos[q1 * 16 + g * 4 + r16];
                    if (te1 >= 0) visit(v1, te1);
                }
            }
        }
    };
    scan([&](float v, int te) {
        if (v >= t) {
            const int slot = atomicAdd(&s_cnt, 1);
            if (slot < LE_CAP) { s_cv[slot] = v; s_cp[slot] = te; }
        }
    });
    __syncthreads();
    if (HGR_LAB_ON(dbg == 4)) return;
    const int cnt = s_cnt;
    if (cnt <= LE_CAP) {
        rank_and_emit<LE_NT>(s_cv, s_cp, cnt, k, tid, [&](int rk, float, int p) { out_topk[(int64_t)row * k + rk] = test_cols[p]; });
        return;
    }
    __syncthreads();
    if (tid == 0) s_ncand = 0;
    __syncthreads();
    for (int q = tid; q < S * LE_GPS; q += LE_NT)
        if (s_gm[q] > -INFINITY && s_gm[q] >= t) s_cand[atomicAdd(&s_ncand, 1)] = (short)q;
    __syncthreads();
    ncand = s_ncand;
    Best last = {INFINITY, -1};
    for (int j = 0; j < k; ++j) {
        Best b = {-INFINITY, 0x7fffffff};
        scan([&](float v, int te) { if (better(last.v, last.p, v, te) && better(v, te, b.v, b.p)) { b.v = v; b.p = te; } });
        last = block_best<LE_NW>(b, s_bv, s_bp, tid);
        if (tid == 0) out_topk[(int64_t)row * k + j] = last.p < n_test ? test_cols[last.p] : -1;
    }
}

}

int hgr_logits_eval_rows_launch(const void *feat, const void *zslp, int D, int S, const unsigned long long *keys, const float *tmax,
                                const int *gp1, const float *gm2, const int32_t *level_first, int n_levels, const int32_t *filler_pos, const int32_t *train_cols, int n_train,
                                const int32_t *epos, const int32_t *test_cols, int n_test, int k, int32_t *out_level, int32_t *out_top1,
                                int32_t *out_topk, int rows, int dtype, void *stream) {
    static int dbg = -1;
    if (dbg < 0) dbg = hgr_lab_env("HGR_LE_DBG");
    if (dtype == HGR_BF16) hipLaunchKernelGGL((logits_eval_rows<HGR_BF16>), dim3(rows), dim3(LE_NT), 0, (hipStream_t)stream, feat, zslp, D, S, keys, tmax, gp1, gm2, level_first,
                                              n_levels, filler_pos, train_cols, n_train, epos, test_cols, n_test, k, out_level, out_top1, out_topk, dbg, rows);
    else hipLaunchKernelGGL((logits_eval_rows<HGR_F16>), dim3(rows), dim3(LE_NT), 0, (hipStream_t)stream, feat, zslp, D, S, keys, tmax, gp1, gm2, level_first,
                            n_levels, filler_pos, train_cols, n_train, epos, test_cols, n_test, k, out_level, out_top1, out_topk, dbg, rows);
    HGR_CHECK_LAUNCH("hgr_logits_eval (row stage)");
    return HGR_OK;
}

extern "C" int hgr_topk_rows(const float *logits, int64_t ld, const int32_t *cols, int n_cols, int k,
                             int32_t *out_idx, float *out_val, int rows, void *stream) {
    HGR_REQUIRE(logits && out_idx, "hgr_topk_rows: null operand");
    HGR_REQUIRE(rows >= 1 && n_cols >= 1 && n_cols <= 40000 && k >= 1 && k <= 32 && k <= n_cols,
                "hgr_topk_rows: rows=%d n_cols=%d k=%d unsupported (n_cols <= 40000, k <= min(32, n_cols))", rows, n_cols, k);
    HGR_REQUIRE(ld >= 1, "hgr_topk_rows: bad ld");
    static size_t granted = 0;
    const size_t bytes = ((size_t)n_cols * 4 + 15) & ~(size_t)15;
    if (bytes > granted) {
        hipError_t e = hipFuncSetAttribute((const void *)topk_rows, hipFuncAttributeMaxDynamicSharedMemorySize, (int)bytes);
        if (e != hipSuccess) return hgr_set_error(HGR_ELAUNCH, "hgr_topk_rows: cannot reserve %zu B of LDS: %s", bytes, hipGetErrorString(e));
        granted = bytes;
    }
    hipLaunchKernelGGL(topk_rows, dim3(rows), dim3(256), bytes, (hipStream_t)stream, logits, ld, cols, n_cols, k, out_idx, out_val);
    HGR_CHECK_LAUNCH("hgr_topk_rows");
    return HGR_OK;
}

extern "C" int hgr_level_argmax(const float *logits, int64_t ld, const int32_t *cols, int n_cols,
                                const int32_t *depth, int n_levels, int32_t *out, int32_t *out_top1, int rows, void *stream) {
    HGR_REQUIRE(logits && depth && out, "hgr_level_argmax: null operand");
    HGR_REQUIRE(rows >= 1 && n_cols >= 1 && n_levels >= 1 && n_levels <= 32, "hgr_level_argmax: rows=%d n_cols=%d n_levels=%d unsupported (n_levels <= 32)", rows, n_cols, n_levels);
    hipStream_t s = (hipStream_t)stream;
    if (n_levels <= 16) hipLaunchKernelGGL((level_argmax<16>), dim3(rows), dim3(256), 0, s, logits, ld, cols, n_cols, depth, n_levels, out, out_top1);
    else hipLaunchKernelGGL((level_argmax<32>), dim3(rows), dim3(256), 0, s, logits, ld, cols, n_cols, depth, n_levels, out, out_top1);
    HGR_CHECK_LAUNCH("hgr_level_argmax");
    return HGR_OK;
}

namespace {
__global__ __launch_bounds__(1024) void eval_counters(const int32_t *__restrict__ pred, int k, const int64_t *__restrict__ targets, int target,
                                                      const int32_t *__restrict__ top1, const int32_t *__restrict__ lv, int n_levels,
                                                      const int32_t *__restrict__ parents, const int32_t *__restrict__ levels, int L,
                                                      double *__restrict__ acc, int B) {
    __shared__ unsigned s_red[16][8];
    __shared__ int s_par[32], s_lev[32];
    if (threadIdx.x < 32) {
        s_par[threadIdx.x] = threadIdx.x < L ? parents[threadIdx.x] : -1;
        s_lev[threadIdx.x] = threadIdx.x < L ? levels[threadIdx.x] : 0;
    }
    __syncthreads();
    unsigned cnt[8] = {0, 0, 0, 0, 0, 0, 0, 0};
    for (int r = threadIdx.x; r < B; r += 1024) {
        const int tgt = targets ? (int)targets[r] : target;
        int pr[32], lvv[32];
#pragma unroll
        for (int i = 0; i < 32; ++i) pr[i] = i < k ? pred[(int64_t)r * k + i] : -1;
#pragma unroll
        for (int i = 0; i < 32; ++i) lvv[i] = i < L ? lv[(int64_t)r * n_levels + s_lev[i]] : -1;
        const int t1 = top1[r];
        int j = k;
#pragma unroll
        for (int i = 31; i >= 0; --i)
            if (i < k && pr[i] == tgt) j = i;
        cnt[0] += j < 1; cnt[1] += j < 2; cnt[2] += j < 5; cnt[3] += j < 10; cnt[4] += j < 20;
        bool prev = false;
#pragma unroll
        for (int i = 0; i < 32; ++i) {
            const int pa = s_par[i];
            const bool live = i < L;
            cnt[5] += live && t1 == pa;
            const bool m = live && lvv[i] == pa;
            cnt[7] += m;
            if (L == 1) cnt[6] += m;
            else if (i > 0) cnt[6] += (m && prev);
            prev = m;
        }
    }
#pragma unroll
    for (int c = 0; c < 8; ++c) {
        unsigned v = cnt[c];
#pragma unroll
        for (int o = 32; o > 0; o >>= 1) v += __shfl_xor(v, o);
        if ((threadIdx.x & 63) == 0) s_red[threadIdx.x >> 6][c] = v;
    }
    __syncthreads();
    if (threadIdx.x == 0) {
        unsigned t[8];
        for (int c = 0; c < 8; ++c) {
            t[c] = 0;
            for (int w = 0; w < 16; ++w) t[c] += s_red[w][c];
        }
        for (int c = 0; c < 6; ++c) acc[c] += (double)t[c];
        acc[6] += L > 1 ? (double)t[6] / (double)(L - 1) : (double)t[6];
        acc[7] += (double)t[7] / (double)L;
        acc[8] += (double)B;
    }
}
}

extern "C" int hgr_eval_counters(const int32_t *pred, int k, const int64_t *targets, int target, const int32_t *top1, const int32_t *lv,
                                 int n_levels, const int32_t *parents, const int32_t *levels, int L, double *acc, int rows, void *stream) {
    HGR_REQUIRE(pred && top1 && lv && parents && levels && acc, "hgr_eval_counters: null operand");
    HGR_REQUIRE(rows >= 1 && k >= 1 && k <= 32 && L >= 1 && L <= 32 && n_levels >= 1, "hgr_eval_counters: bad sizes rows=%d k=%d L=%d (k, L <= 32)", rows, k, L);
    hipLaunchKernelGGL(eval_counters, dim3(1), dim3(1024), 0, (hipStream_t)stream, pred, k, targets, target, top1, lv, n_levels, parents, levels, L, acc, rows);
    HGR_CHECK_LAUNCH("hgr_eval_counters");
    return HGR_OK;
}

extern "C" int hgr_eval_rows(const float *logits, int64_t ld, int n_nodes, const unsigned char *lvl8, const int32_t *train_pos,
                             const int32_t *train_cols, int n_train, int n_levels, const int32_t *filler_pos, const int32_t *test_pos,
                             const int32_t *test_cols, int n_test, int k, int32_t *out_level, int32_t *out_top1, int32_t *out_topk,
                             int rows, void *stream) {
    HGR_REQUIRE(logits && lvl8 && train_pos && train_cols && filler_pos && out_level, "hgr_eval_rows: null operand");
    HGR_REQUIRE(rows >= 1 && n_nodes >= 1 && ld >= n_nodes && n_train >= 1 && n_levels >= 1 && n_levels <= 32, "hgr_eval_rows: bad sizes (n_levels <= 32)");
    HGR_REQUIRE(k == 0 || (out_topk && test_pos && test_cols && k >= 1 && k <= 32 && n_test >= k), "hgr_eval_rows: bad top-k arguments");
    if (n_levels <= EL_NLV) hipLaunchKernelGGL(eval_rows_lds, dim3(rows), dim3(EL_NT), 0, (hipStream_t)stream, logits, ld, n_nodes, lvl8, train_pos, train_cols,
                                               n_train, n_levels, filler_pos, test_pos, test_cols, n_test, k, out_level, out_top1, out_topk);
    else hipLaunchKernelGGL(eval_rows, dim3(rows), dim3(EV_NT), 0, (hipStream_t)stream, logits, ld, n_nodes, lvl8, train_pos, train_cols, n_train,
                            n_levels, filler_pos, test_pos, test_cols, n_test, k, out_level, out_top1, out_topk);
    HGR_CHECK_LAUNCH("hgr_eval_rows");
    return HGR_OK;
}
```

### hgr-net_amd/model/clip_tree.py

```python
from __future__ import annotations

import copy
import math
import os
import random
from typing import Optional, Sequence

import torch
import torch.nn as nn

from .. import clip, ops
from ..graphs import GraphCache
from ..hierarchy import build_hierarchy
from .._lib import HgrError

TEMPLATE = "a photo of a {}."

TAIL_OVERLAP = os.environ.get("HGR_TAIL_OVERLAP", "1") != "0"
LOGITS_SPLIT = os.environ.get("HGR_LOGITS_SPLIT", "class")


class _StopHead(Exception):
    """Raised by the split hook while the HEAD graph of a pipelined step is captured: the rest of the step belongs to the tail graph."""


def _classifier_part(slot: str):
    def fget(self):
        return self.__dict__.get(slot)

    def fset(self, value):
        self.__dict__[slot] = value
        self.__dict__["_cls_token"] = self.__dict__.get("_cls_token", 0) + 1
    return property(fget, fset)


class _Pipe:

    def __init__(self, dev):
        self.side = torch.cuda.Stream(device=dev, priority=int(os.environ.get("HGR_TAIL_PRIO", "-1")))
        self.cache = GraphCache(8, "all", pre_drop=self.drain)
        self.ok = None
        self.step = 0
        self.head_done = [torch.cuda.Event(), torch.cuda.Event()]
        self.tail_done = [torch.cuda.Event(), torch.cuda.Event()]
        for e in self.tail_done:
            e.record()

    def drain(self) -> None:
        main = torch.cuda.current_stream()
        main.wait_stream(self.side)
        main.synchronize()


class tree_model(nn.Module):
    zsl_weights = _classifier_part("_cls_zsl32")
    _zsl16 = _classifier_part("_cls_zsl16")

    def __init__(self, opts, candidates_train: Sequence[str], candidates_test: Sequence[str],
                 node_tokens: Optional[torch.Tensor] = None, clip_model: Optional[nn.Module] = None):
        super().__init__()
        self.opts = opts
        self.device = f"cuda:{opts.device}" if isinstance(opts.device, int) else opts.device
        self.save_path = "{}/{}/{}_{}_{}/".format(opts.folder, opts.exp_name, opts.weights, opts.out_ratio, opts.in_ratio)
        self.file_path = self.save_path + "clip_{}".format(opts.from_epoch)
        os.makedirs(self.save_path, exist_ok=True)

        import json
        with open(opts.graph_path, "r") as f:
            self.hierarchy = build_hierarchy(json.load(f))
        self.p2c, self.c2p, self.d2n, self.nodes, self.start_up = self.hierarchy.as_tuple()
        self.nodes_id = list(range(len(self.nodes)))

        if clip_model is None:
            clip_model, _ = clip.load(name=opts.arch, device=self.device, download_root="pretrained",
                                      image_dtype=getattr(opts, "image_dtype", "f16"),
                                      text_dtype=getattr(opts, "text_dtype", "f16"))
        self.clip_model = clip_model
        if getattr(opts, "fetch", False):
            self.clip_model.load_state_dict(torch.load(opts.fetch_path, map_location=self.device))
        if getattr(opts, "load", False):
            path = self.file_path if opts.load_path == "none" else opts.load_path
            self.clip_model.load_state_dict(torch.load(path, map_location=self.device))
            print("successfully loaded")
        self.clip_model.eval()
        for p in self.clip_model.parameters():
            p.requires_grad_(True)
        self.loss = nn.CrossEntropyLoss()

        self.n_ctx = int(getattr(opts, "n_ctx", 0) or 0)
        if node_tokens is None:
            tmpl = (" ".join(["X"] * self.n_ctx) + " {}.") if self.n_ctx else TEMPLATE
            node_tokens = clip.tokenize([tmpl.format(self._wordnet_name(n)) for n in self.nodes])
        self.ctx = None
        if self.n_ctx:
            wt = self.clip_model.transformer.width
            self.ctx = nn.Parameter(torch.empty(self.n_ctx, wt, device=self.device).normal_(std=0.02))
        if node_tokens.shape[0] != len(self.nodes):
            raise ValueError(f"node_tokens has {node_tokens.shape[0]} rows for {len(self.nodes)} nodes")
        self.node_tokens = node_tokens.long().to(self.device)

        self.resolution = self.clip_model.visual.input_resolution
        self.candidates_train, self.candidates_test = candidates_train, candidates_test
        index = {n: i for i, n in enumerate(self.nodes)}
        self.train_index = torch.tensor([index[c] for c in candidates_train]).to(self.device)
        self.test_index = torch.tensor([index[c] for c in candidates_test]).to(self.device)
        self.max_depth = max(self.d2n.keys())
        if opts.weights == "adaptive":
            num_layer = [len(self.d2n[layer]) for layer in self.d2n.keys()]
            self.layer_weight = nn.Parameter(((1.0 / torch.tensor(num_layer, dtype=torch.float32)) * opts.scale).to(self.device))

        self.train_index32 = self.train_index.to(torch.int32)
        self.test_index32 = self.test_index.to(torch.int32)
        self.depth32 = torch.from_numpy(self.hierarchy.depth).to(self.device)
        self.zsl_weights = None
        self._zsl16 = None
        self.use_graph = os.environ.get("HGR_GRAPH", "1") != "0"
        self._graph_cache = GraphCache(4, "oldest")
        self._pipe = None

    @staticmethod
    def _wordnet_name(wnid: str) -> str:
        try:
            from nltk.corpus import wordnet as wn
        except Exception as e:
            raise RuntimeError("WordNet (nltk) is not available: pass node_tokens= to tree_model") from e
        return wn.synset_from_pos_and_offset("n", int(wnid[1:])).name().split(".")[0].replace("_", " ")

    def save(self, opts, epoch):
        torch.save(self.clip_model.state_dict(), self.save_path + "clip_{}".format(epoch))

    @torch.no_grad()
    def update_classifier(self, group=None):
        n = len(self.nodes)
        if group is not None:
            from ..parallel import sharded_text_features
            feats = sharded_text_features(self.clip_model, self.node_tokens, group, ctx=self.ctx)
        else:
            feats = self.clip_model.encode_text(self.node_tokens, ctx=self.ctx)
        z32 = torch.empty_like(feats)
        z16 = torch.empty(feats.shape, dtype=self.clip_model.image_dtype, device=feats.device)
        ops.l2norm_rows(feats, y16=z16, y32=z32)
        self.zsl_weights, self._zsl16 = z32, z16
        assert z32.shape[0] == n

    @torch.no_grad()
    def forward(self, inputs, targets=None, static_output: bool = False):
        if self._zsl16 is None:
            raise HgrError("call update_classifier() before forward()")
        self.join_tail()
        if self.use_graph and inputs.is_cuda:
            return self._forward_graphed(inputs, static_output)
        return self._forward_eager(inputs)

    @torch.no_grad()
    def forward_eval(self, inputs, plan, k: int):
        if self._zsl16 is None:
            raise HgrError("call update_classifier() before forward_eval()")
        self.join_tail()
        plan.bind(self._eval_class_operand(), self._zsl16.shape[1])
        if self.use_graph and inputs.is_cuda:
            return self._forward_graphed(inputs, True, ("eval", plan, k))
        return self._forward_eager(inputs, ("eval", plan, k))

    def _generation(self, inputs, mode):
        cm = self.clip_model
        return (tuple(inputs.shape), inputs.dtype, self._cls_token, cm._ws.epoch, cm._fingerprint(), tuple(sorted(cm._ln_off)), mode)

    def _forward_graphed(self, inputs, static_output: bool = False, mode=None):
        self.clip_model.poll_ln_guard()
        cache = self._graph_cache
        if cache.renew(self._generation(inputs, mode)):
            self._forward_eager(inputs, mode)
            cache.gen = self._generation(inputs, mode)
        g, out = cache.lookup(inputs, 0, lambda buf, slot: self._capture(buf, mode))
        g.replay()
        return out if (static_output or mode is not None) else out.clone()

    def _eager_phase(self, inputs, mode, phase: str, tag: str):
        from .. import _lib
        seen = []
        if phase == "head":
            def hook(name):
                seen.append(name)
                raise _StopHead()
        else:
            def hook(name):
                seen.append(name)
                _lib.set_muted(False)
        prev_hook, prev_tag = ops.SPLIT_HOOK, self.clip_model._img_tag
        ops.SPLIT_HOOK, self.clip_model._img_tag = hook, tag
        out = None
        try:
            _lib.set_muted(phase == "tail")
            out = self._forward_eager(inputs, mode)
        except _StopHead:
            pass
        finally:
            _lib.set_muted(False)
            ops.SPLIT_HOOK, self.clip_model._img_tag = prev_hook, prev_tag
        return out, bool(seen)

    def _pipe_state(self, dev) -> _Pipe:
        if self._pipe is None:
            self._pipe = _Pipe(dev)
        return self._pipe

    def join_tail(self) -> None:
        if self._pipe is not None:
            torch.cuda.current_stream().wait_stream(self._pipe.side)

    @torch.no_grad()
    def forward_eval_overlapped(self, inputs, plan, k: int, consume) -> bool:
        if not (TAIL_OVERLAP and self.use_graph and inputs.is_cuda) or self._zsl16 is None:
            return False
        if inputs.dtype not in (torch.float32, torch.uint8) or not inputs.is_contiguous():
            return False
        from ..clip import model as _clip_model
        if _clip_model.IMG_STREAMS > 1:
            return False
        plan.bind(self._eval_class_operand(), self._zsl16.shape[1])
        mode = ("eval", plan, k)
        st = self._pipe_state(inputs.device)
        self.clip_model.poll_ln_guard()
        main = torch.cuda.current_stream()
        if self._generation(inputs, mode) != st.cache.gen:
            main.wait_stream(st.side)
            ok = True
            for tag in ("v", "v@1"):
                ok &= self._eager_phase(inputs, mode, "head", tag)[1]
                if ok:
                    self._eager_phase(inputs, mode, "tail", tag)
            main.synchronize()
            st.cache.renew(self._generation(inputs, mode))
            st.ok = ok
        if not st.ok:
            return False
        par = st.step & 1
        st.step += 1

        def capture(buf, par):
            tag = "v@1" if par else "v"
            epoch = self.clip_model._ws.epoch
            st.drain()
            gh, gt = torch.cuda.CUDAGraph(), torch.cuda.CUDAGraph()
            with torch.cuda.graph(gh):
                self._eager_phase(buf, mode, "head", tag)
            with torch.cuda.graph(gt):
                outs, _ = self._eager_phase(buf, mode, "tail", tag)
            if epoch != self.clip_model._ws.epoch:
                raise HgrError("workspace buffers moved during the capture of a pipelined evaluation step")
            return gh, gt, outs
        gh, gt, outs = st.cache.lookup(inputs, par, capture)
        main.wait_event(st.tail_done[par])
        gh.replay()
        st.head_done[par].record(main)
        with torch.cuda.stream(st.side):
            st.side.wait_event(st.head_done[par])
            gt.replay()
            consume(*outs)
            st.tail_done[par].record(st.side)
        return True

    def _capture(self, inputs, mode=None):
        self._forward_eager(inputs, mode)
        torch.cuda.current_stream().synchronize()
        g = torch.cuda.CUDAGraph()
        with torch.cuda.graph(g):
            out = self._forward_eager(inputs, mode)
        return g, out

    def _eval_class_operand(self):
        split = LOGITS_SPLIT if (LOGITS_SPLIT in ("class", "feat") and 2 * self._zsl16.shape[1] <= 1024) else ""
        if not split:
            return self._zsl16
        key = (split, self._cls_token)
        if getattr(self, "_zsl_split_key", None) != key:
            z16 = self._zsl16
            second = (self.zsl_weights.float() - z16.float()).to(z16.dtype) if split == "class" else z16
            self._zsl_split, self._zsl_split_key = torch.cat([z16, second], dim=1).contiguous(), key
        return self._zsl_split

    def _forward_eager(self, inputs, mode=None):
        feats = self.clip_model.encode_image(inputs)
        b, n = feats.shape[0], self._zsl16.shape[0]
        f16 = torch.empty(feats.shape, dtype=self._zsl16.dtype, device=feats.device)
        zc = self._eval_class_operand() if mode is None else mode[1].zsl
        if zc is not None and zc.shape[1] == 2 * feats.shape[1]:
            if LOGITS_SPLIT == "feat":
                f32 = torch.empty_like(feats)
                ops.l2norm_rows(feats, y16=f16, y32=f32)
                second = (f32 - f16.float()).to(f16.dtype)
            else:
                ops.l2norm_rows(feats, y16=f16)
                second = f16
            fin = torch.cat([f16, second], dim=1)
        else:
            ops.l2norm_rows(feats, y16=f16)
            fin, zc = f16, (self._zsl16 if mode is None else zc)
        if mode is not None:
            return ops.logits_eval(fin, mode[1], mode[2])
        ld = (n + 63) // 64 * 64
        logits = torch.empty((b, ld), dtype=torch.float32, device=feats.device)
        ops.gemm_nt(fin, zc, logits, n=n, tag="logits")
        return logits[:, :n]

    def get_contra_ids(self, method, target, depth=None, parents=None):
        nc = self.opts.num_compare
        if method == "random":
            ids = random.sample(self.train_index.tolist(), nc)
        elif method == "topk":
            low, high = min(self.d2n.keys()), max(self.d2n.keys())
            if depth - self.opts.k > low:
                low = depth - self.opts.k
            cand = []
            for d in range(low, depth):
                cand.extend(self.d2n[d])
            if depth == 0:
                cand.extend(self.d2n[depth])
            ids = list(set(cand) - set(parents))
            if len(ids) > nc:
                ids = random.sample(ids, nc)
        elif method == "brothers":
            if len(parents) > 1 and depth > 0:
                ids = copy.copy(self.p2c[parents[depth - 1]])
            else:
                ids = copy.copy(self.start_up)
            if len(ids) > nc:
                ids = random.sample(ids, nc)
        elif method == "near_simi":
            low, high = min(self.d2n.keys()), max(self.d2n.keys())
            low = max(low, depth - self.opts.k)
            high = min(high, depth + self.opts.k)
            cand = set()
            for d in range(low, high + 1):
                cand.update(self.d2n[d])
            cand = sorted(cand - set(parents) - set(self.p2c[target]) - {target})
            nc = min(nc, len(cand))
            with torch.no_grad():
                toks = self.node_tokens[torch.tensor([target] + cand, device=self.node_tokens.device)]
                f = self.clip_model.encode_text(toks, ctx=self.ctx.data if self.ctx is not None else None).float()
                f = f / f.norm(dim=-1, keepdim=True)
                order = (f[1:] @ f[0]).argsort(descending=True, stable=True)[:nc].tolist()
            ids = [cand[i] for i in order]
        else:
            raise NotImplementedError(f"sample_strategy {method!r} (the reference's 'simi' reads attributes that do not exist)")
        if target not in ids:
            ids.append(target)
        return ids, ids.index(target)

    def get_weights(self, method, max_depth=None, device=None):
        dev = self.device if device is None else device
        if method == "equal":
            return (torch.ones(max_depth) / max_depth).to(dev)
        if method == "decreasing":
            w = torch.arange(start=max_depth, end=0, step=-1).to(dev)
        elif method == "increasing":
            w = torch.arange(start=1, end=max_depth + 1).to(dev)
        elif method == "nl_increasing":
            w = (torch.arange(start=1, end=max_depth + 1) ** 3).to(dev)
        elif method == "nl_decreasing":
            w = (torch.arange(start=max_depth, end=0, step=-1) ** 3).to(dev)
        elif method == "adaptive":
            return torch.softmax(100 ** self.layer_weight[:max_depth], dim=0)
        else:
            raise ValueError(method)
        return w / w.sum()

    def outer_inner_plan(self, target: int):
        parents = copy.copy(self.c2p[target]) + [target]
        k = max(1, math.ceil(self.opts.out_ratio * len(parents)))
        outer = parents[::-1][:k]
        plan = []
        for k_loop, p_out in enumerate(outer):
            parents_in = copy.copy(self.c2p[p_out]) + [p_out]
            m = max(1, math.ceil(self.opts.in_ratio * len(parents_in)))
            inner = parents_in[::-1][:m]
            for m_loop, p_in in enumerate(inner):
                plan.append(dict(p_out=p_out, p_in=p_in, depth=parents_in.index(p_in), parents_in=parents_in,
                                 k_loop=k_loop, m_loop=m_loop, K=len(outer), M=len(inner)))
        return plan

    def train_batch(self, inputs, targets, training_method, sample_strategy):
        if getattr(self, "_trainer", None) is None:
            from ..training import OMTrainer
            self._trainer = OMTrainer(self, getattr(self.opts, "train_dtype", "bf16"))
        return self._trainer.train_batch(inputs, targets, training_method, sample_strategy)
```

### hgr-net_amd/ops.py

```python
from __future__ import annotations

import math
from typing import Optional

import torch

from . import _lib
from ._lib import (EPI_ACCUM, EPI_BIAS, EPI_BIAS_ADD16_RELU, EPI_BIAS_QUICKGELU, EPI_BIAS_RELU, EPI_BIAS_RESIDUAL, EPI_NONE, EPI_QGELU_GRAD16,
                   HGR_BF16, HGR_F16)

PROFILE = None

WEIGHTS_GEN = [0]

SPLIT_HOOK = None


def split_point(name: str) -> None:
    h = SPLIT_HOOK
    if h is not None:
        h(name)


TORCH16 = {HGR_BF16: torch.bfloat16, HGR_F16: torch.float16}
# ... 277 lines not shown


def vit_embed_ln(patches, cls, pos, gamma, beta, x, b, g, eps=1e-5):
    _lib.call("hgr_vit_embed_ln", _dev(patches), _dev(cls), _dev(pos), _dev(gamma), _dev(beta), _dev(x), b, g, x.shape[1], eps, _stream())
    return x


def layernorm(x: torch.Tensor, gamma, beta, out: torch.Tensor, rows: Optional[int] = None, row_mul: int = 1,
              row_idx: Optional[torch.Tensor] = None, eps: float = 1e-5) -> torch.Tensor:
    w = x.shape[-1]
    rows = out.shape[0] if rows is None else rows
    out32 = out.dtype == torch.float32
    _lib.call("hgr_layernorm", _dev(x), _dev(gamma), _dev(beta), _dev(out), rows, w, row_mul, _dev(row_idx), eps,
              HGR_BF16 if out32 else DT_OF[out.dtype], 1 if out32 else 0, _stream())
    return out


def mha(qkv: torch.Tensor, out: torch.Tensor, b: int, l: int, heads: int, causal: bool, stats: Optional[torch.Tensor] = None,
        q_rows: int = 0) -> torch.Tensor:
    assert qkv.is_contiguous() and out.is_contiguous() and qkv.shape[1] == 3 * heads * 64 and out.shape[1] == heads * 64
    if q_rows:
        assert stats is None
        _lib.call("hgr_mha_rows", _dev(qkv), _dev(out), b, l, heads, 1 if causal else 0, int(q_rows), DT_OF[qkv.dtype], _stream())
        return out
    if stats is not None:
        assert stats.dtype == torch.float32 and stats.is_contiguous() and stats.numel() == b * heads * l * 2
        _lib.call("hgr_mha_stats", _dev(qkv), _dev(out), _dev(stats), b, l, heads, 1 if causal else 0, DT_OF[qkv.dtype], _stream())
        return out
    _lib.call("hgr_mha", _dev(qkv), _dev(out), b, l, heads, 1 if causal else 0, DT_OF[qkv.dtype], _stream())
    return out


def text_embed(tokens: torch.Tensor, emb: torch.Tensor, pos: torch.Tensor, x: torch.Tensor, l: int) -> torch.Tensor:
    assert tokens.dtype == torch.int64 and tokens.stride(1) == 1
    n = tokens.shape[0]
    _lib.call("hgr_text_embed", _dev(tokens), tokens.stride(0), _dev(emb), _dev(pos), _dev(x), n, l, emb.shape[1], emb.shape[0], _stream())
    return x


def eot_index(tokens: torch.Tensor, out: torch.Tensor) -> torch.Tensor:
    assert tokens.dtype == torch.int64 and out.dtype == torch.int32
    _lib.call("hgr_eot_index", _dev(tokens), tokens.stride(0), _dev(out), tokens.shape[0], tokens.shape[1], _stream())
    return out


def l2norm_rows(x: torch.Tensor, y16: Optional[torch.Tensor] = None, y32: Optional[torch.Tensor] = None) -> None:
    assert x.dtype == torch.float32 and x.is_contiguous()
    dt = DT_OF[y16.dtype] if y16 is not None else HGR_BF16
    _lib.call("hgr_l2norm_rows", _dev(x), _dev(y16), _dev(y32), x.shape[0], x.shape[1], dt, _stream())


def topk_rows(logits: torch.Tensor, k: int, cols: Optional[torch.Tensor] = None, n_cols: Optional[int] = None,
              want_values: bool = False):
    assert logits.dtype == torch.float32 and logits.stride(1) == 1
    rows = logits.shape[0]
    nc = cols.numel() if cols is not None else (logits.shape[1] if n_cols is None else n_cols)
    idx = torch.empty((rows, k), dtype=torch.int32, device=logits.device)
    val = torch.empty((rows, k), dtype=torch.float32, device=logits.device) if want_values else None
    _lib.call("hgr_topk_rows", _dev(logits), logits.stride(0), _dev(cols), nc, k, _dev(idx), _dev(val), rows, _stream())
    return (idx, val) if want_values else idx


def level_argmax(logits: torch.Tensor, depth: torch.Tensor, n_levels: int, cols: Optional[torch.Tensor] = None,
                 n_cols: Optional[int] = None, want_top1: bool = False):
    assert logits.dtype == torch.float32 and logits.stride(1) == 1 and depth.dtype == torch.int32
    rows = logits.shape[0]
    nc = cols.numel() if cols is not None else (logits.shape[1] if n_cols is None else n_cols)
    out = torch.empty((rows, n_levels), dtype=torch.int32, device=logits.device)
    top1 = torch.empty((rows, 1), dtype=torch.int32, device=logits.device) if want_top1 else None
    _lib.call("hgr_level_argmax", _dev(logits), logits.stride(0), _dev(cols), nc, _dev(depth), n_levels, _dev(out), _dev(top1), rows, _stream())
    return (out, top1) if want_top1 else out


class EvalIndex:

    def __init__(self, depth: torch.Tensor, train_cols: torch.Tensor, test_cols: Optional[torch.Tensor], n_levels: int):
        import numpy as np
        d = depth.cpu().numpy()
        n = len(d)
        tr = train_cols.cpu().numpy().astype(np.int64)
        assert d.min() >= 0 and n_levels <= 32 and d[tr].max() < n_levels, "a subset node lies deeper than n_levels"
        assert len(set(tr.tolist())) == len(tr), "train columns must be distinct"
        lv = d[tr]
        filler = np.full(n_levels, -1, dtype=np.int32)
        for l in range(n_levels):
            other = np.nonzero(lv != l)[0]
            if other.size:
                filler[l] = int(other[0])
        tpos = np.full(n, -1, dtype=np.int32)
        tpos[tr] = np.arange(len(tr), dtype=np.int32)
        dev = depth.device
        self.n_nodes, self.n_levels, self.n_train = n, n_levels, len(tr)
        self.lvl8 = torch.from_numpy(np.minimum(d, 255).astype(np.uint8)).to(dev)
        self.train_pos = torch.from_numpy(tpos).to(dev)
        self.train_cols = train_cols.to(torch.int32).contiguous()
        self.filler = torch.from_numpy(filler).to(dev)
        self.test_pos = self.test_cols = None
        self.n_test = 0
        if test_cols is not None:
            te = test_cols.cpu().numpy().astype(np.int64)
            assert len(set(te.tolist())) == len(te), "test columns must be distinct"
            epos = np.full(n, -1, dtype=np.int32)
            epos[te] = np.arange(len(te), dtype=np.int32)
            self.test_pos = torch.from_numpy(epos).to(dev)
            self.test_cols = test_cols.to(torch.int32).contiguous()
            self.n_test = len(te)


def eval_rows(logits: torch.Tensor, index: EvalIndex, k: int):
    assert logits.dtype == torch.float32 and logits.stride(1) == 1 and logits.shape[1] >= index.n_nodes
    rows = logits.shape[0]
    dev = logits.device
    lvl = torch.empty((rows, index.n_levels), dtype=torch.int32, device=dev)
    top1 = torch.empty((rows, 1), dtype=torch.int32, device=dev)
    topk = torch.empty((rows, max(k, 1)), dtype=torch.int32, device=dev)
    _lib.call("hgr_eval_rows", _dev(logits), logits.stride(0), index.n_nodes, _dev(index.lvl8), _dev(index.train_pos), _dev(index.train_cols),
              index.n_train, index.n_levels, _dev(index.filler), _dev(index.test_pos), _dev(index.test_cols), index.n_test, k,
              _dev(lvl), _dev(top1), _dev(topk), rows, _stream())
    return lvl, top1, topk


class LogitsEvalPlan:
    SLICE, SLAB = 32, 96

    def __init__(self, index: EvalIndex):
        import numpy as np
        lvl = index.lvl8.cpu().numpy().astype(np.int64)
        tpos = index.train_pos.cpu().numpy()
        epos = index.test_pos.cpu().numpy() if index.test_pos is not None else np.full(len(lvl), -1, dtype=np.int32)
        cols, level_first = [], [0]
        for l in range(index.n_levels):
            c = np.nonzero(lvl == l)[0]
            pad = (-c.size) % self.SLICE
            cols.append(np.concatenate([c, np.full(pad, -1, dtype=np.int64)]))
            level_first.append(level_first[-1] + (c.size + pad) // self.SLICE)
        assert int((lvl >= index.n_levels).sum()) == 0, "a node lies deeper than n_levels"
        perm = np.concatenate(cols)
        tail = (-perm.size) % self.SLAB
        if tail or perm.size == 0:
            perm = np.concatenate([perm, np.full(tail or self.SLAB, -1, dtype=np.int64)])
        dev = index.lvl8.device
        valid = perm >= 0
        safe = np.where(valid, perm, 0)
        self.index = index
        self.n_perm = int(perm.size)
        self.perm = torch.from_numpy(safe).to(dev)
        self.valid = torch.from_numpy(valid).to(dev)
        self.tpos = torch.from_numpy(np.where(valid, tpos[safe], -1).astype(np.int32)).to(dev)
        self.epos = torch.from_numpy(np.where(valid, epos[safe], -1).astype(np.int32)).to(dev)
        self.level_first = torch.from_numpy(np.asarray(level_first, dtype=np.int32)).to(dev)
        self.zsl = None
        self._src = None
        self._ws = None

    MAX_SLICES = 1024

    @property
    def supported(self) -> bool:
        return self.n_perm // self.SLICE <= self.MAX_SLICES and self.index.n_levels <= 32

    def bind(self, zsl16: torch.Tensor, algo_d: Optional[int] = None) -> "LogitsEvalPlan":
        self.algo_d = int(algo_d or zsl16.shape[1])
        if self._src is not zsl16:
            z = zsl16[self.perm]
            z[~self.valid] = 0
            self.zsl, self._src = z.contiguous(), zsl16
        return self

    def workspace(self, rows: int, dev) -> torch.Tensor:
        need = int(_lib.load().hgr_logits_eval_workspace_bytes(rows, self.n_perm))
        if self._ws is None or self._ws.numel() < need or self._ws.device != torch.device(dev):
            self._ws = torch.empty(need, dtype=torch.uint8, device=dev)
        return self._ws


def logits_eval(feat16: torch.Tensor, plan: LogitsEvalPlan, k: int, stage: str = ""):
    ix = plan.index
    assert plan.zsl is not None, "LogitsEvalPlan.bind(zsl16) first"
    assert feat16.is_contiguous() and feat16.dtype == plan.zsl.dtype and feat16.shape[1] == plan.zsl.shape[1]
    rows, d = feat16.shape
    dev = feat16.device
    lvl = torch.empty((rows, ix.n_levels), dtype=torch.int32, device=dev)
    top1 = torch.empty((rows, 1), dtype=torch.int32, device=dev)
    topk = torch.empty((rows, max(k, 1)), dtype=torch.int32, device=dev)
    prof = PROFILE
    ev = _prof_begin()
    _lib.call({"": "hgr_logits_eval", "tile": "hgr_logits_eval_tile_stage", "row": "hgr_logits_eval_row_stage"}[stage],
              _dev(feat16), _dev(plan.zsl), rows, d, plan.n_perm, _dev(plan.tpos), _dev(plan.epos), _dev(plan.level_first),
              ix.n_levels, _dev(ix.filler), _dev(ix.train_cols), ix.n_train, _dev(ix.test_cols), ix.n_test, k,
              _dev(lvl), _dev(top1), _dev(topk), _dev(plan.workspace(rows, dev)), DT_OF[feat16.dtype], _stream())
    da = getattr(plan, "algo_d", d)
    _prof_end(ev, 2.0 * rows * ix.n_nodes * da, 2 * rows * da + 2 * ix.n_nodes * da, "logits_eval" + ("_" + stage if stage else ""))
    return lvl, top1, topk


def eval_counters(pred: torch.Tensor, targets: Optional[torch.Tensor], target: int, top1: torch.Tensor, lv: torch.Tensor,
                  parents: torch.Tensor, levels: torch.Tensor, acc: torch.Tensor) -> None:
    assert pred.dtype == top1.dtype == lv.dtype == parents.dtype == levels.dtype == torch.int32 and acc.dtype == torch.float64
    assert pred.is_contiguous() and lv.is_contiguous() and top1.is_contiguous() and acc.numel() == 9
    assert targets is None or (targets.dtype == torch.int64 and targets.is_contiguous() and targets.numel() == pred.shape[0])
    _lib.call("hgr_eval_counters", _dev(pred), pred.shape[1], _dev(targets), int(target), _dev(top1), _dev(lv), lv.shape[1], _dev(parents),
              _dev(levels), parents.numel(), _dev(acc), pred.shape[0], _stream())


def eval_counters_rows(pred: torch.Tensor, targets: torch.Tensor, top1: torch.Tensor, lv: torch.Tensor, anc_ptr: torch.Tensor,
                       anc_nodes: torch.Tensor, anc_levels: torch.Tensor, acc: torch.Tensor) -> None:
    assert pred.dtype == top1.dtype == lv.dtype == anc_ptr.dtype == anc_nodes.dtype == anc_levels.dtype == torch.int32 and acc.dtype == torch.float64
    assert pred.is_contiguous() and lv.is_contiguous() and top1.is_contiguous() and acc.numel() == 9
    assert anc_ptr.is_contiguous() and anc_nodes.is_contiguous() and anc_levels.is_contiguous() and anc_ptr.numel() >= 2
    assert targets is not None and targets.dtype == torch.int64 and targets.is_contiguous() and targets.numel() == pred.shape[0]
    assert top1.numel() == pred.shape[0] and lv.shape[0] == pred.shape[0]
    _lib.call("hgr_eval_counters_rows", _dev(pred), pred.shape[1], _dev(targets), _dev(top1), _dev(lv), lv.shape[1], _dev(anc_ptr),
              _dev(anc_nodes), _dev(anc_levels), anc_ptr.numel() - 1, _dev(acc), pred.shape[0], _stream())


REPORT_MAXL = 32
REPORT_DEPTH_COLS = ("rows", "hit@1", "hit@2", "hit@5", "hit@10", "hit@20", "anc_hit", "point", "edge", "chain")
REPORT_DEPTH = 0
REPORT_LEVEL = REPORT_DEPTH + (REPORT_MAXL + 1) * len(REPORT_DEPTH_COLS)
REPORT_DIST_BINS = 2 * REPORT_MAXL + 2
REPORT_DIST_UNKNOWN = 2 * REPORT_MAXL + 1
REPORT_DIST_TEST = REPORT_LEVEL + 2 * REPORT_MAXL
REPORT_DIST_ALL = REPORT_DIST_TEST + REPORT_DIST_BINS
REPORT_HEIGHT = REPORT_DIST_ALL + REPORT_DIST_BINS
REPORT_HEIGHT_K = (1, 2, 5, 10, 20)
REPORT_LEN = REPORT_HEIGHT + len(REPORT_HEIGHT_K)


def eval_report_rows(pred: torch.Tensor, targets: torch.Tensor, top1: torch.Tensor, lv: torch.Tensor, anc_ptr: torch.Tensor,
                     anc_nodes: torch.Tensor, anc_levels: torch.Tensor, table: torch.Tensor) -> None:
    assert pred.dtype == top1.dtype == lv.dtype == anc_ptr.dtype == anc_nodes.dtype == anc_levels.dtype == torch.int32
    assert table.dtype == torch.int64 and table.numel() == REPORT_LEN and table.is_contiguous()
    assert pred.is_contiguous() and lv.is_contiguous() and top1.is_contiguous()
    assert anc_ptr.is_contiguous() and anc_nodes.is_contiguous() and anc_levels.is_contiguous() and anc_ptr.numel() >= 2
    assert targets is not None and targets.dtype == torch.int64 and targets.is_contiguous() and targets.numel() == pred.shape[0]
    assert top1.numel() == pred.shape[0] and lv.shape[0] == pred.shape[0]
    _lib.call("hgr_eval_report_rows", _dev(pred), pred.shape[1], _dev(targets), _dev(top1), _dev(lv), lv.shape[1], _dev(anc_ptr),
              _dev(anc_nodes), _dev(anc_levels), anc_ptr.numel() - 1, _dev(table), pred.shape[0], _stream())


PATH_MAXL = 32


def path_scores(logits: torch.Tensor, anc_ptr: torch.Tensor, anc_nodes: torch.Tensor, wtab: torch.Tensor,
                out: Optional[torch.Tensor] = None) -> torch.Tensor:
    n_nodes = anc_ptr.numel() - 1
    assert logits.dim() == 2 and logits.dtype == torch.float32 and logits.stride(1) == 1 and logits.shape[1] >= n_nodes >= 1
    assert anc_ptr.dtype == anc_nodes.dtype == torch.int32 and anc_ptr.is_contiguous() and anc_nodes.is_contiguous()
    assert wtab.dtype == torch.float32 and wtab.shape == (PATH_MAXL + 1, PATH_MAXL) and wtab.is_contiguous()
    rows = logits.shape[0]
    if out is None:
        out = torch.empty((rows, n_nodes), dtype=torch.float32, device=logits.device)
    assert out.dim() == 2 and out.dtype == torch.float32 and out.stride(1) == 1 and out.shape[0] == rows and out.shape[1] >= n_nodes
    _lib.call("hgr_path_scores", _dev(logits), logits.stride(0), _dev(out), out.stride(0), n_nodes, _dev(anc_ptr), _dev(anc_nodes),
              _dev(wtab), rows, _stream())
    return out[:, :n_nodes]


HEDGE_MAXT = 8
HEDGE_MAXN = 36864
HEDGE_SCALE = 1 << 30
HEDGE_COL_NAMES = ("rows", "abstain", "exact", "ancestor", "below", "wrong", "sum_lpick", "sum_common", "sum_lt")
HEDGE_COL_HIST = len(HEDGE_COL_NAMES)
HEDGE_COLS = HEDGE_COL_HIST + REPORT_MAXL + 1


def hedge_thresholds(thetas) -> list:
    try:
        th = [float(t) for t in thetas]
    except TypeError:
        raise ValueError(f"hedge thresholds {thetas!r}: a sequence of numbers") from None
    if not 1 <= len(th) <= HEDGE_MAXT:
        raise ValueError(f"hedge: {len(th)} thresholds (1..{HEDGE_MAXT})")
    if not all(0.0 < t <= 1.0 for t in th):
        raise ValueError(f"hedge thresholds {th}: each in (0, 1]")
    if any(b <= a for a, b in zip(th, th[1:])):
        raise ValueError(f"hedge thresholds {th}: strictly increasing")
    return [int(math.ceil(t * HEDGE_SCALE)) for t in th]


def subtree_hedge(scores: torch.Tensor, cand_pos: Optional[torch.Tensor], anc_ptr: torch.Tensor, anc_nodes: torch.Tensor,
                  temperature: float, thr: torch.Tensor, pick: Optional[torch.Tensor] = None, pick_mass: Optional[torch.Tensor] = None,
                  mass_out: Optional[torch.Tensor] = None):
    n_nodes = anc_ptr.numel() - 1
    assert scores.dim() == 2 and scores.dtype == torch.float32 and scores.stride(1) == 1
    assert anc_ptr.dtype == anc_nodes.dtype == torch.int32 and anc_ptr.is_contiguous() and anc_nodes.is_contiguous()
    assert cand_pos is None or (cand_pos.dtype == torch.int32 and cand_pos.is_contiguous() and cand_pos.numel() == n_nodes)
    assert thr.dtype == torch.int32 and thr.dim() == 1 and thr.is_contiguous()
    rows, t = scores.shape[0], thr.numel()
    if pick is None:
        pick = torch.empty((rows, t), dtype=torch.int32, device=scores.device)
    if pick_mass is None:
        pick_mass = torch.empty((rows, t), dtype=torch.float32, device=scores.device)
    assert pick.dtype == torch.int32 and pick.shape == (rows, t) and pick.is_contiguous()
    assert pick_mass.dtype == torch.float32 and pick_mass.shape == (rows, t) and pick_mass.is_contiguous()
    assert mass_out is None or (mass_out.dim() == 2 and mass_out.dtype == torch.int32 and mass_out.stride(1) == 1 and mass_out.shape[0] == rows)
    _lib.call("hgr_subtree_hedge", _dev(scores), scores.stride(0), n_nodes, _dev(cand_pos), _dev(anc_ptr), _dev(anc_nodes), float(temperature),
              _dev(thr), t, _dev(pick), _dev(pick_mass), _dev(mass_out), mass_out.stride(0) if mass_out is not None else 0, rows, _stream())
    return pick, pick_mass


def hedge_counters_rows(pick: torch.Tensor, targets: torch.Tensor, anc_ptr: torch.Tensor, anc_nodes: torch.Tensor, table: torch.Tensor) -> None:
    assert pick.dtype == anc_ptr.dtype == anc_nodes.dtype == torch.int32 and pick.dim() == 2 and pick.is_contiguous()
    assert anc_ptr.is_contiguous() and anc_nodes.is_contiguous() and anc_ptr.numel() >= 2
    assert table.dtype == torch.int64 and table.shape == (pick.shape[1], HEDGE_COLS) and table.is_contiguous()
    assert targets is not None and targets.dtype == torch.int64 and targets.is_contiguous() and targets.numel() == pick.shape[0]
    _lib.call("hgr_hedge_counters_rows", _dev(pick), pick.shape[1], _dev(targets), _dev(anc_ptr), _dev(anc_nodes), anc_ptr.numel() - 1,
              _dev(table), pick.shape[0], _stream())


SETS_MAXS = 16
SETS_COL_NAMES = ("rows", "hit@1", "hit@2", "hit@5", "hit@10", "hit@20", "anc_hit", "point", "edge")
SETS_COLS = len(SETS_COL_NAMES)


def check_sets(sets, n_nodes: int) -> dict:
    try:
        items = [(str(k), [int(c) for c in (v.tolist() if hasattr(v, "tolist") else v)]) for k, v in dict(sets).items()]
    except (TypeError, ValueError):
        raise ValueError(f"sets {sets!r}: a mapping from a name to node ids") from None
    if not 1 <= len(items) <= SETS_MAXS:
        raise ValueError(f"sets: {len(items)} candidate sets (1..{SETS_MAXS})")
    for name, ids in items:
        if len(set(ids)) != len(ids):
            raise ValueError(f"sets[{name!r}]: a node id appears twice")
        bad = [c for c in ids if not 0 <= c < n_nodes]
        if bad:
            raise ValueError(f"sets[{name!r}]: node id {bad[0]} outside the hierarchy (0..{n_nodes - 1})")
    return dict(items)


class SetIndex:

    def __init__(self, eval_index: EvalIndex, sets):
        import numpy as np
        n = eval_index.n_nodes
        items = list(check_sets(sets, n).items())
        member = np.zeros(n, dtype=np.int32)
        for s, (name, ids) in enumerate(items):
            member[np.asarray(ids, dtype=np.int64)] |= np.int32(1 << s)
        key = np.full(n, -1, dtype=np.int64)
        if eval_index.test_pos is not None:
            key = eval_index.test_pos.cpu().numpy().astype(np.int64)
        rest = key < 0
        key[rest] = eval_index.n_test + np.arange(int(rest.sum()), dtype=np.int64)
# ... 479 lines not shown
```

### include/hgr.h

```cpp
#ifndef HGR_H
#define HGR_H

#include <stdint.h>

#ifdef __cplusplus
extern "C" {
#endif

#define HGR_ABI_VERSION 5

enum { HGR_OK = 0, HGR_EINVAL = -1, HGR_EUNSUPPORTED = -2, HGR_ELAUNCH = -3 };

typedef enum { HGR_BF16 = 0, HGR_F16 = 1 } hgr_dtype_t;

typedef enum {
    HGR_EPI_NONE = 0,
    HGR_EPI_BIAS = 1,
    HGR_EPI_BIAS_QUICKGELU = 2,
    HGR_EPI_BIAS_RESIDUAL = 3,
    HGR_EPI_BIAS_RELU = 4,
    HGR_EPI_BIAS_ADD16_RELU = 5,
    HGR_EPI_ACCUM = 6,
    HGR_EPI_QGELU_GRAD16 = 7
} hgr_epilogue_t;
// ... 141 lines not shown

int hgr_transpose16(const void *x, int64_t ldx, void *y, int64_t ldy, int rows, int cols, void *stream);

int hgr_transpose16_colsum(const void *x, int64_t ldx, void *y, int64_t ldy, int rows, int cols, int dtype,
                           float *out, int accumulate, float alpha, float *scratch, void *stream);

int hgr_colsum(const void *x, int64_t ldx, int rows, int cols, int x_f32, int dtype, float *out, int accumulate,
               float alpha, float *scratch, void *stream);

int hgr_cast16(const float *x, void *y, int64_t n, int dtype, void *stream);
int hgr_cast16_transpose(const float *x, int64_t ldx, void *y, int64_t ldy, void *yt, int64_t ldyt, int rows, int cols, int dtype, void *stream);

int hgr_quickgelu16(const void *a, const void *du, void *out, int64_t n, int backward, int dtype, void *stream);

int hgr_layernorm_bwd(const void *dy, int dy_f32, const float *x, const float *gamma, float *dx, float *dgamma,
                      float *dbeta, float *scratch, int rows, int W, int64_t row_mul, const int32_t *row_idx,
                      float eps, int dtype, void *stream);
int hgr_layernorm_bwd_cast(const void *dy, int dy_f32, const float *x, const float *gamma, float *dx, void *dx16, float *dgamma,
                           float *dbeta, float *scratch, int rows, int W, int64_t row_mul, const int32_t *row_idx, float eps,
                           int dtype, void *stream);
int hgr_layernorm_bwd_cast_colsum(const void *dy, int dy_f32, const float *x, const float *gamma, float *dx, void *dx16, float *dgamma,
                                  float *dbeta, float *dx16_colsum, float *scratch, int rows, int W, int64_t row_mul,
                                  const int32_t *row_idx, float eps, int dtype, void *stream);
int64_t hgr_layernorm_bwd_scratch_floats(int rows, int W);

int hgr_mha_bwd(const void *qkv, const void *out, const void *dout, void *dqkv, int B, int L, int heads, int causal, int dtype, void *stream);
int hgr_mha_bwd_stats(const void *qkv, const void *out, const void *dout, void *dqkv, const float *stats,
                      int B, int L, int heads, int causal, int dtype, void *stream);
int hgr_mha_bwd_colsum(const void *qkv, const void *out, const void *dout, void *dqkv, const float *stats, float *colsum_part,
                       int B, int L, int heads, int causal, int dtype, void *stream);

int hgr_conv3x3_nhwc_plain(const void *x, const void *w, void *out, int B, int H, int W, int C, int Cout, int Kp,
                           int dtype, void *stream);
int hgr_gemm_nt_splitk(const void *A, int64_t lda, const void *W, int64_t ldw, float *partial, int64_t ldc,
                       int M, int N, int K, int kc, int dtype, void *stream);
int hgr_relu_bwd16(const void *dy, const void *y, void *out, int64_t n, int dtype, void *stream);
int hgr_add16(const void *a, const void *b, void *out, int64_t n, int dtype, void *stream);
int hgr_avgpool2_bwd_nhwc(const void *dy, void *dx, int B, int H, int W, int C, int dtype, void *stream);
int hgr_attnpool_tokens_bwd(const void *dtok, void *dx, int B, int S, int C, int dtype, void *stream);
int hgr_im2col3x3_t(const void *xt, void *out, int B, int H, int W, int C, int64_t ld, int dtype, void *stream);
int hgr_bn_fold(const float *w, const float *gamma, const float *beta, const float *mean, const float *var, float eps,
                void *w16, float *bias, int Cout, int Cin, int khw, int Kp, int dtype, void *stream);
int hgr_bn_unfold_grad(const float *gwf, int64_t ldg, const float *gbf, const float *w, const float *gamma, const float *mean,
                       const float *var, float eps, float *g_w, float *g_gamma, float *g_beta, int Cout, int Cin, int khw,
                       void *stream);

int hgr_csr_group_aggregate(const float *support, int64_t ld_support, const int *item_row, const int *item_e0,
                            const int *item_e1, const int *item_slot, int n_items, const int *col, const float *inv_deg,
                            const unsigned char *grp, const float *att, int D, const float *bias,
                            const int *split_row, const int *split_slot0, const int *split_n, int n_split,
                            float *partial, float *out, int64_t ld_out, int C, float slope, int normalize, void *stream);

int hgr_csr_group_att_grad(const float *support, int64_t ld_support, const float *bias, const float *g, int64_t ld_g,
                           const float *y, int64_t ld_y, float *dout, int64_t ld_dout, const int *item_row,
                           const int *item_e0, const int *item_e1, const int *item_slot, int n_items, const int *col,
                           const float *inv_deg, const unsigned char *grp, int D, const int *split_row,
                           const int *split_slot0, const int *split_n, int n_split, float *partial, float *P, int C,
                           float slope, void *stream);

int hgr_dgp_loss_head(const float *O, int64_t ld_o, const int *rows, const float *F, int64_t ld_f, int n_t, int n,
                      float *loss_rows, float *loss, float *dout, int64_t ld_dout, int C, void *stream);

int hgr_dropout_counter(const float *x, int64_t ld_x, float *y, int64_t ld_y, int rows, int C, int seed, int step, int layer,
                        void *stream);

int hgr_adam_l2(float *p, const float *g, float *m, float *v, int64_t n, float lr, float beta1, float beta2, float eps, float wd,
                int step, void *stream);

int hgr_cnzsl_std_chain_fwd(const float *z, int64_t ld_z, const float *bias, float *running_mean1, float *running_var1,
                            float *running_mean2, float *running_var2, float *c, int64_t ld_c, float *a, int64_t ld_a,
                            float *stats, int S, int H, int train, float eps, float momentum, void *stream);

int hgr_cnzsl_std_chain_bwd(const float *dc, int64_t ld_dc, const float *a, int64_t ld_a, const float *z, int64_t ld_z,
                            const float *bias, const float *stats, float *dz, int64_t ld_dz, float *dbias, int S, int H,
                            float eps, void *stream);

int hgr_bias_relu_f32(const float *x, int64_t ld_x, const float *bias, float *y, int64_t ld_y, int rows, int C, void *stream);

int hgr_relu_bwd_colsum_f32(const float *dy, int64_t ld_dy, const float *y, int64_t ld_y, float *dx, int64_t ld_dx, float *db,
                            float *scratch, int rows, int C, void *stream);

int hgr_ce_rows(const float *logits, int64_t ld, const int32_t *labels, int rows, int n, float gscale,
                float *loss_rows, float *dlogits, int64_t ldd, void *stream);

int hgr_l2norm_bwd(const float *x, const float *dy, float *dx, int rows, int D, int accumulate, void *stream);

int hgr_matmul_f32(const float *A, int64_t sam, int64_t sak, const float *B, int64_t sbk, int64_t sbn, float *C,
                   int64_t ldc, int M, int N, int K, float alpha, int accumulate, void *stream);

int hgr_dot_f32(const float *a, const float *b, int64_t n, float *out, float alpha, int accumulate, void *stream);

int hgr_embed_scatter_add(const int64_t *tokens, int64_t ld_tokens, const float *dx, float *dtable, int n, int L,
                          int W, int vocab, void *stream);

int hgr_rows_axpy(float *dst, int64_t dst_mul, const int32_t *dst_idx, const float *src, int rows, int W, float alpha, void *stream);

int hgr_ctx_splice(float *x, const float *ctx, const float *positional_embedding, int n, int L, int W, int n_ctx, void *stream);
int hgr_ctx_splice_bwd(float *dx, float *dctx, int n, int L, int W, int n_ctx, void *stream);

int hgr_rows_gather(float *dst, const float *src, const int32_t *idx, int rows, int W, void *stream);

int hgr_sumsq(const float *x, int64_t n, float *out, void *stream);

int hgr_adamw(float *p, const float *g, float *m, float *v, int64_t n, float lr, float beta1, float beta2, float eps,
              float wd, int step, const float *sumsq_total, float max_norm, float grad_scale, void *stream);

int hgr_gemm_nt_res_stats(const void *A, int64_t lda, const void *W, int64_t ldw, void *xh, void *xl, int64_t ldx,
                          const float *bias, float *stats, int M, int N, int K, int dtype, void *stream);

int hgr_gemm_nt_res_stats_guard(const void *A, int64_t lda, const void *W, int64_t ldw, void *xh, void *xl, int64_t ldx,
                                const float *bias, float *stats, float guard_sumsq, uint32_t *flag,
                                int M, int N, int K, int dtype, void *stream);

int hgr_vit_head(const void *xh, const void *xl, int64_t ldx, int64_t row_mul, const float *gamma, const float *beta, float eps,
                 const void *proj_t, float *out, int B, int W, int D, int dtype, void *stream);
int hgr_gemm_nt_ln(const void *XH, int64_t ldx, const void *Wfold, int64_t ldw, void *C, int64_t ldc,
                   const float *ln_s, const float *ln_c, const float *stats, float eps,
                   int M, int N, int K, int dtype, int act, void *stream);

int hgr_gemm_nt_ln_mha(const void *XH, int64_t ldx, const void *Wfold, int64_t ldw, const float *ln_s, const float *ln_c,
                       const float *stats, float eps, void *att, int64_t ldatt, int B, int L, int heads, int causal,
                       int dtype, void *stream);

int hgr_gemm_nt_bias_gelu_dual(const void *A, int64_t lda, const void *W, int64_t ldw, void *pre, int64_t ldpre, void *post, int64_t ldpost,
                               const float *bias, int M, int N, int K, int dtype, void *stream);
int hgr_gemm_nt_qgelu_grad_colsum(const void *A, int64_t lda, const void *W, int64_t ldw, void *C, int64_t ldc, const void *pre, int64_t ldpre,
                                  float *colsum_part, int M, int N, int K, int dtype, void *stream);
int hgr_vit_embed_ln_stats(const float *patches, const float *class_embedding, const float *positional_embedding,
                           const float *gamma, const float *beta, void *xh, void *xl, float *stats,
                           int B, int G, int W, float eps, int dtype, void *stream);
int hgr_vit_patch_embed_ln_ok(int B, int R, int P, int W, int dtype);
int hgr_vit_patch_embed_ln(const float *image, const void *conv_w, const float *class_embedding, const float *positional_embedding,
                           const float *gamma, const float *beta, void *xh, void *xl, float *stats,
                           int B, int R, int P, int W, float eps, int dtype, void *stream);
int hgr_row_stats16(const float *x, void *xh, void *xl, float *stats, int rows, int W, int dtype, void *stream);
int hgr_pair_rows_f32(const void *xh, const void *xl, float *out, int rows, int W, int64_t row_mul, const int32_t *row_idx, int dtype, void *stream);

int64_t hgr_logits_eval_workspace_bytes(int rows, int n_perm);
int hgr_logits_eval(const void *feat16, const void *zsl_perm16, int rows, int D, int n_perm,
                    const int32_t *tpos_perm, const int32_t *epos_perm, const int32_t *level_first,
                    int n_levels, const int32_t *filler_pos, const int32_t *train_cols, int n_train,
                    const int32_t *test_cols, int n_test, int k,
                    int32_t *out_level, int32_t *out_top1, int32_t *out_topk, void *workspace, int dtype, void *stream);
int hgr_logits_eval_tile_stage(const void *feat16, const void *zsl_perm16, int rows, int D, int n_perm,
                    const int32_t *tpos_perm, const int32_t *epos_perm, const int32_t *level_first,
                    int n_levels, const int32_t *filler_pos, const int32_t *train_cols, int n_train,
                    const int32_t *test_cols, int n_test, int k,
                    int32_t *out_level, int32_t *out_top1, int32_t *out_topk, void *workspace, int dtype, void *stream);
int hgr_logits_eval_row_stage(const void *feat16, const void *zsl_perm16, int rows, int D, int n_perm,
                    const int32_t *tpos_perm, const int32_t *epos_perm, const int32_t *level_first,
                    int n_levels, const int32_t *filler_pos, const int32_t *train_cols, int n_train,
                    const int32_t *test_cols, int n_test, int k,
                    int32_t *out_level, int32_t *out_top1, int32_t *out_topk, void *workspace, int dtype, void *stream);

#define HGR_COMM_ID_BYTES 128
typedef enum { HGR_COMM_F32 = 0, HGR_COMM_F64 = 1, HGR_COMM_F16 = 2, HGR_COMM_BF16 = 3, HGR_COMM_I32 = 4, HGR_COMM_I64 = 5, HGR_COMM_U8 = 6 } hgr_comm_dtype_t;
typedef enum { HGR_COMM_SUM = 0, HGR_COMM_MAX = 1 } hgr_comm_op_t;

int hgr_comm_unique_id(void *id_out );
int hgr_comm_init(int rank, int world, const void *unique_id );
int hgr_comm_destroy(void);
int hgr_comm_rank(void);
int hgr_comm_world(void);
int hgr_allreduce(const void *send, void *recv, int64_t count, int dtype, int op, void *stream);
int hgr_allgather(const void *send, void *recv, int64_t count_per_rank, int dtype, void *stream);
int hgr_broadcast(void *buf, int64_t count, int dtype, int root, void *stream);

#ifdef __cplusplus
}
#endif
#endif
```

Before: 107,200.

## Evaluate split-precision class logits using only the high half with bounded fallback

When class embeddings are stored as hi/lo split halves, the slab GEMM now computes logits from the hi half only and records top-two values per slice. The row stage uses a precomputed error bound (dcoef times the feature norm) to decide which candidates could change ranking and rescores only those with the full hi+lo product, counting fallback rows. This is meant to avoid the second K pass over the lo half or a separate split path, roughly halving logits GEMM work. In exchange it adds more per-slice bookkeeping, extra shared memory in the row kernel, and relies on the bound being conservative enough to keep hit@1 parity.

After: 107,300 (median of 2 runs). Within noise of the previous version (+0.1%).

```diff
diff --git a/hgr-net_amd/_lib.py b/hgr-net_amd/_lib.py
--- a/hgr-net_amd/_lib.py
+++ b/hgr-net_amd/_lib.py
@@ -114,6 +114,9 @@
     "hgr_logits_eval": [_p, _p, _i, _i, _i, _p, _p, _p, _i, _p, _p, _i, _p, _i, _i, _p, _p, _p, _p, _i, _p],
     "hgr_logits_eval_tile_stage": [_p, _p, _i, _i, _i, _p, _p, _p, _i, _p, _p, _i, _p, _i, _i, _p, _p, _p, _p, _i, _p],
     "hgr_logits_eval_row_stage": [_p, _p, _i, _i, _i, _p, _p, _p, _i, _p, _p, _i, _p, _i, _i, _p, _p, _p, _p, _i, _p],
+    "hgr_logits_eval_split": [_p, _p, _i, _i, _i, _p, _p, _p, _i, _p, _p, _i, _p, _i, _i, _p, _p, _p, _p, _i, _p, _f, _p],
+    "hgr_logits_eval_split_tile_stage": [_p, _p, _i, _i, _i, _p, _p, _p, _i, _p, _p, _i, _p, _i, _i, _p, _p, _p, _p, _i, _p, _f, _p],
+    "hgr_logits_eval_split_row_stage": [_p, _p, _i, _i, _i, _p, _p, _p, _i, _p, _p, _i, _p, _i, _i, _p, _p, _p, _p, _i, _p, _f, _p],
     "hgr_comm_unique_id": [_p],
     "hgr_comm_init": [_i, _i, _p],
     "hgr_comm_destroy": [],
diff --git a/hgr-net_amd/csrc/hgr_gemm.hip b/hgr-net_amd/csrc/hgr_gemm.hip
--- a/hgr-net_amd/csrc/hgr_gemm.hip
+++ b/hgr-net_amd/csrc/hgr_gemm.hip
@@ -442,15 +442,18 @@
     int32_t *out_level, int32_t *out_top1, int32_t *out_topk, void *workspace, int dtype, void *stream
 #define HGR_LE_ARGS feat16, zsl_perm16, rows, D, n_perm, tpos_perm, epos_perm, level_first, n_levels, filler_pos, train_cols, n_train, test_cols, n_test, k, \
     out_level, out_top1, out_topk, workspace, dtype, stream
-static int logits_eval_stages(int stages, HGR_LE_PARAMS);
+static int logits_eval_stages(int stages, HGR_LE_PARAMS, bool split = false, float dcoef = 0.f, int32_t *fallback_rows = nullptr);
 extern "C" int hgr_logits_eval(HGR_LE_PARAMS) { return logits_eval_stages(3, HGR_LE_ARGS); }
+extern "C" int hgr_logits_eval_split(HGR_LE_PARAMS, float dcoef, int32_t *fallback_rows) { return logits_eval_stages(3, HGR_LE_ARGS, true, dcoef, fallback_rows); }
+extern "C" int hgr_logits_eval_split_tile_stage(HGR_LE_PARAMS, float dcoef, int32_t *fallback_rows) { return logits_eval_stages(1, HGR_LE_ARGS, true, dcoef, fallback_rows); }
+extern "C" int hgr_logits_eval_split_row_stage(HGR_LE_PARAMS, float dcoef, int32_t *fallback_rows) { return logits_eval_stages(2, HGR_LE_ARGS, true, dcoef, fallback_rows); }
 extern "C" int hgr_logits_eval_tile_stage(HGR_LE_PARAMS) { return logits_eval_stages(1, HGR_LE_ARGS); }
 extern "C" int hgr_logits_eval_row_stage(HGR_LE_PARAMS) { return logits_eval_stages(2, HGR_LE_ARGS); }
 
 int hgr_logits_eval_rows_launch(const void *feat, const void *zslp, int D, int S, const unsigned long long *keys, const float *tmax,
                                 const int *gp1, const float *gm2, const int32_t *level_first, int n_levels, const int32_t *filler_pos, const int32_t *train_cols, int n_train,
                                 const int32_t *epos, const int32_t *test_cols, int n_test, int k, int32_t *out_level, int32_t *out_top1,
-                                int32_t *out_topk, int rows, int dtype, void *stream);
+                                int32_t *out_topk, int rows, int dtype, void *stream, const int32_t *tpos, float dcoef, int *fallback_rows);
 
 extern "C" int64_t hgr_logits_eval_workspace_bytes(int rows, int n_perm) {
     if (rows < 1 || n_perm < 96 || n_perm % 96) return -1;
@@ -461,7 +464,8 @@
                                const int32_t *tpos_perm, const int32_t *epos_perm, const int32_t *level_first,
                                int n_levels, const int32_t *filler_pos, const int32_t *train_cols, int n_train,
                                const int32_t *test_cols, int n_test, int k,
-                               int32_t *out_level, int32_t *out_top1, int32_t *out_topk, void *workspace, int dtype, void *stream) {
+                               int32_t *out_level, int32_t *out_top1, int32_t *out_topk, void *workspace, int dtype, void *stream,
+                               bool split, float dcoef, int32_t *fallback_rows) {
     HGR_REQUIRE(feat16 && zsl_perm16 && tpos_perm && epos_perm && level_first && filler_pos && train_cols && out_level && workspace, "hgr_logits_eval: null operand");
     HGR_REQUIRE(rows >= 1 && D >= 128 && D % 128 == 0 && D <= 1024, "hgr_logits_eval: rows=%d D=%d unsupported (D %% 128 == 0, D <= 1024)", rows, D);
     HGR_REQUIRE(n_perm >= 96 && n_perm % 96 == 0 && n_perm / 32 <= 1024, "hgr_logits_eval: n_perm=%d must be a multiple of 96 and <= 32768 (32-column level-aligned slices, 96-column slabs)", n_perm);
@@ -469,10 +473,12 @@
     HGR_REQUIRE(k == 0 || (out_topk && test_cols && k >= 1 && k <= 32 && n_test >= k), "hgr_logits_eval: bad top-k arguments");
     HGR_REQUIRE(hgr_aligned(feat16, 16) && hgr_aligned(zsl_perm16, 16) && hgr_aligned(tpos_perm, 16) && hgr_aligned(epos_perm, 16) && hgr_aligned(workspace, 16), "hgr_logits_eval: operands must be 16-byte aligned");
     HGR_REQUIRE(dtype == HGR_BF16 || dtype == HGR_F16, "hgr_logits_eval: bad dtype %d", dtype);
-    HGR_REQUIRE((int64_t)rows * D * 2 < (1ll << 32) && (int64_t)n_perm * D * 2 < (1ll << 32), "hgr_logits_eval: operands beyond 4 GB");
+    HGR_REQUIRE(!split || (D <= 512 && dcoef >= 0.f && dcoef < INFINITY), "hgr_logits_eval_split: D=%d dcoef=%g unsupported (D <= 512: class rows of 2 D <= 1024; finite dcoef >= 0)", D, (double)dcoef);
+    const int ldz = split ? 2 * D : D;
+    HGR_REQUIRE((int64_t)rows * D * 2 < (1ll << 32) && (int64_t)n_perm * ldz * 2 < (1ll << 32), "hgr_logits_eval: operands beyond 4 GB");
     const int S = n_perm / 32;
     SlabArgs a;
-    a.A = (const char *)feat16; a.lda = D; a.W = (const char *)zsl_perm16; a.ldw = D; a.M = rows; a.K = D; a.Np = n_perm;
+    a.A = (const char *)feat16; a.lda = D; a.W = (const char *)zsl_perm16; a.ldw = ldz; a.M = rows; a.K = D; a.Np = n_perm; a.hi_only = split;
     a.tpos = tpos_perm; a.epos = epos_perm; a.S = S;
     { static const int d = hgr_lab_env("HGR_LS_DBG"); a.dbg = d; }
     a.ev_key = (unsigned long long *)workspace;
@@ -483,5 +489,5 @@
     HGR_CHECK_LAUNCH("hgr_logits_eval (tile stage)");
     if (!(stages & 2)) return HGR_OK;
     return hgr_logits_eval_rows_launch(feat16, zsl_perm16, D, S, a.ev_key, a.ev_tmax, a.ev_p1, a.ev_m2, level_first, n_levels, filler_pos, train_cols, n_train,
-                                       epos_perm, test_cols, n_test, k, out_level, out_top1, out_topk, rows, dtype, stream);
-}
+                                       epos_perm, test_cols, n_test, k, out_level, out_top1, out_topk, rows, dtype, stream, split ? tpos_perm : nullptr, dcoef, fallback_rows);
+}
diff --git a/hgr-net_amd/csrc/hgr_gemm_common.h b/hgr-net_amd/csrc/hgr_gemm_common.h
--- a/hgr-net_amd/csrc/hgr_gemm_common.h
+++ b/hgr-net_amd/csrc/hgr_gemm_common.h
@@ -267,6 +267,7 @@
     unsigned long long *ev_key = nullptr;
     float *ev_tmax = nullptr, *ev_m2 = nullptr; int *ev_p1 = nullptr;
     int S = 0;
+    bool hi_only = false;
     int dbg = 0;
 };
 void launch_logits_slab(const SlabArgs &a, int dtype, hipStream_t s);
diff --git a/hgr-net_amd/csrc/hgr_logits_slab.hip b/hgr-net_amd/csrc/hgr_logits_slab.hip
--- a/hgr-net_amd/csrc/hgr_logits_slab.hip
+++ b/hgr-net_amd/csrc/hgr_logits_slab.hip
@@ -6,7 +6,7 @@
 constexpr int LS_NT = 512;
 constexpr int LS_PA0 = 0, LS_PA1 = 32768, LS_PW = 65536, LS_STAGE = 81920, LS_LDS = 2 * LS_STAGE;
 
-template <int DT>
+template <int DT, bool HI>
 __global__ __launch_bounds__(LS_NT) void logits_slab(SlabArgs p) {
     typedef typename T16<DT>::vec8 vec8;
     __shared__ __attribute__((aligned(1024))) char smem[LS_LDS];
@@ -127,6 +127,10 @@
         const int n = n0 + j * 16 + g * 4;
         const int4 t4 = *(const int4 *)(p.tpos + n), e4 = *(const int4 *)(p.epos + n);
         tp[j][0] = t4.x; tp[j][1] = t4.y; tp[j][2] = t4.z; tp[j][3] = t4.w;
+        if constexpr (HI) {
+#pragma unroll
+            for (int e = 0; e < 4; ++e) tp[j][e] = tp[j][e] < 0 ? -1 : (tp[j][e] << 5) | ((j & 1) * 16 + g * 4 + e);
+        }
         ep[j][0] = e4.x; ep[j][1] = e4.y; ep[j][2] = e4.z; ep[j][3] = e4.w;
     }
     char *const rec = (char *)p.ev_key + (int64_t)blockIdx.x * p.M * 96 + g * 24;
@@ -158,16 +162,40 @@
 #pragma unroll
                 for (int e = 0; e < 4; ++e) {
                     tv[jj][e] = tp[2 * s + jj][e] >= 0 ? acc[i][2 * s + jj][e] + 0.0f : -INFINITY;
-                    V = fmaxf(V, tv[jj][e]);
-                }
-            V = xmaxf(V);
+                    if constexpr (!HI) V = fmaxf(V, tv[jj][e]);
+                }
+            float V2 = -INFINITY;
+            if constexpr (HI) {
+                float a1[2], a2[2];
+#pragma unroll
+                for (int jj = 0; jj < 2; ++jj) {
+                    const float hi01 = fmaxf(tv[jj][0], tv[jj][1]), lo01 = fminf(tv[jj][0], tv[jj][1]);
+                    const float hi23 = fmaxf(tv[jj][2], tv[jj][3]), lo23 = fminf(tv[jj][2], tv[jj][3]);
+                    a1[jj] = fmaxf(hi01, hi23);
+                    a2[jj] = fmaxf(fminf(hi01, hi23), fmaxf(lo01, lo23));
+                }
+                V = fmaxf(a1[0], a1[1]);
+                V2 = fmaxf(fminf(a1[0], a1[1]), fmaxf(a2[0], a2[1]));
+                {
+                    auto b1 = LS_SWAP16(__float_as_uint(V)); auto b2 = LS_SWAP16(__float_as_uint(V2));
+                    const float e1 = __uint_as_float(b1[0]), o1 = __uint_as_float(b1[1]);
+                    V2 = fmaxf(fminf(e1, o1), fmaxf(__uint_as_float(b2[0]), __uint_as_float(b2[1])));
+                    V = fmaxf(e1, o1);
+                }
+                {
+                    auto b1 = LS_SWAP32(__float_as_uint(V)); auto b2 = LS_SWAP32(__float_as_uint(V2));
+                    const float e1 = __uint_as_float(b1[0]), o1 = __uint_as_float(b1[1]);
+                    V2 = fmaxf(fminf(e1, o1), fmaxf(__uint_as_float(b2[0]), __uint_as_float(b2[1])));
+                    V = fmaxf(e1, o1);
+                }
+            } else V = xmaxf(V);
             int P = 0x7fffffff;
 #pragma unroll
             for (int jj = 0; jj < 2; ++jj)
 #pragma unroll
                 for (int e = 0; e < 4; ++e) P = min(P, (tp[2 * s + jj][e] >= 0 && tv[jj][e] == V) ? tp[2 * s + jj][e] : 0x7fffffff);
             P = xmini(P);
-            const unsigned long long vkey = key_of(V, P);
+            const unsigned long long vkey = key_of(V, HI ? P >> 5 : P);
             const unsigned long long key = P == 0x7fffffff ? 0ull : vkey;
 #pragma unroll
             for (int jj = 0; jj < 2; ++jj) {
@@ -178,7 +206,8 @@
                 const float hi01 = fmaxf(x[0], x[1]), lo01 = fminf(x[0], x[1]), hi23 = fmaxf(x[2], x[3]), lo23 = fminf(x[2], x[3]);
                 float t1 = fmaxf(hi01, hi23);
                 float t2 = fmaxf(fminf(hi01, hi23), fmaxf(lo01, lo23));
-                int q1 = x[0] == t1 ? ep[j][0] : x[1] == t1 ? ep[j][1] : x[2] == t1 ? ep[j][2] : ep[j][3];
+                int q1 = HI ? g * 4 + (x[0] == t1 ? 0 : x[1] == t1 ? 1 : x[2] == t1 ? 2 : 3)
+                            : x[0] == t1 ? ep[j][0] : x[1] == t1 ? ep[j][1] : x[2] == t1 ? ep[j][2] : ep[j][3];
                 {
                     auto a1 = LS_SWAP16(__float_as_uint(t1)); auto a2 = LS_SWAP16(__float_as_uint(t2)); auto ap = LS_SWAP16(q1);
                     const float e1 = __uint_as_float(a1[0]), o1 = __uint_as_float(a1[1]);
@@ -198,7 +227,8 @@
             if (m < p.M || ((tw[0] ^ tw[1] ^ tw[2]) + (tw[3] ^ tw[4] ^ tw[5]) + ta == 0x9E3779B9u && m == 0x7fffffff)) {
                 const unsigned long long v8 = g == 0 ? key
                     : g == 1 ? ((unsigned long long)__float_as_uint(m1[1]) << 32) | __float_as_uint(m1[0])
-                    : g == 2 ? ((unsigned long long)(unsigned)p1[1] << 32) | (unsigned)p1[0]
+                    : g == 2 ? (HI ? ((unsigned long long)__float_as_uint(V2) << 32) | (unsigned)(p1[0] | ((P & 31) << 8) | (p1[1] << 16))
+                                   : ((unsigned long long)(unsigned)p1[1] << 32) | (unsigned)p1[0])
                              : ((unsigned long long)__float_as_uint(m2[1]) << 32) | __float_as_uint(m2[0]);
                 *(unsigned long long *)(rec + (int64_t)m * 96 + s * 8) = v8;
             }
@@ -211,8 +241,11 @@
 
 void launch_logits_slab(const SlabArgs &a, int dtype, hipStream_t s) {
     const dim3 grid((unsigned)(a.Np / 96), (unsigned)((a.M + 511) / 512)), block(LS_NT);
-    if (dtype == HGR_BF16) hipLaunchKernelGGL((logits_slab<HGR_BF16>), grid, block, 0, s, a);
-    else hipLaunchKernelGGL((logits_slab<HGR_F16>), grid, block, 0, s, a);
-}
-
-}
+    if (a.hi_only) {
+        if (dtype == HGR_BF16) hipLaunchKernelGGL((logits_slab<HGR_BF16, true>), grid, block, 0, s, a);
+        else hipLaunchKernelGGL((logits_slab<HGR_F16, true>), grid, block, 0, s, a);
+    } else if (dtype == HGR_BF16) hipLaunchKernelGGL((logits_slab<HGR_BF16, false>), grid, block, 0, s, a);
+    else hipLaunchKernelGGL((logits_slab<HGR_F16, false>), grid, block, 0, s, a);
+}
+
+}
diff --git a/hgr-net_amd/csrc/hgr_select.hip b/hgr-net_amd/csrc/hgr_select.hip
--- a/hgr-net_amd/csrc/hgr_select.hip
+++ b/hgr-net_amd/csrc/hgr_select.hip
@@ -78,6 +78,13 @@
         last = b;
         __syncthreads();
     }
+}
+
+__device__ __forceinline__ float lowered(float t, float d) {
+    const float r = t - d;
+    if (!(r > -INFINITY)) return r;
+    const unsigned u = __float_as_uint(r);
+    return r > 0.f ? __uint_as_float(u - 1) : r < 0.f ? __uint_as_float(u + 1) : -1.401298464e-45f;
 }
 
 constexpr int TOPK_CAND = 1024;
@@ -410,16 +417,17 @@
 }
 
 
-constexpr int LE_NT = 512, LE_NW = LE_NT / 64, LE_MAXS = 1024, LE_CAP = 2048, LE_GPS = 2;
-
-template <int DT>
+constexpr int LE_NT = 512, LE_NW = LE_NT / 64, LE_MAXS = 1024, LE_CAP = 2048, LE_GPS = 2, LE_SCAP = 256;
+
+template <int DT, bool SPLIT>
 __global__ __launch_bounds__(LE_NT, 4) void logits_eval_rows(const void *__restrict__ feat, const void *__restrict__ zslp, int D, int S,
                                                         const unsigned long long *__restrict__ keys, const float *__restrict__ gmax,
                                                         const int *__restrict__ gp1, const float *__restrict__ gm2,
                                                         const int32_t *__restrict__ level_first, int n_levels, const int32_t *__restrict__ filler_pos,
                                                         const int32_t *__restrict__ train_cols, int n_train, const int32_t *__restrict__ epos,
                                                         const int32_t *__restrict__ test_cols, int n_test, int k,
-                                                        int32_t *__restrict__ out_level, int32_t *__restrict__ out_top1, int32_t *__restrict__ out_topk, int dbg, int rows) {
+                                                        int32_t *__restrict__ out_level, int32_t *__restrict__ out_top1, int32_t *__restrict__ out_topk, int dbg, int rows,
+                                                        const int32_t *__restrict__ tpos, float dcoef, int *__restrict__ fallback_rows) {
     typedef typename T16<DT>::vec8 vec8;
     typedef typename T16<DT>::elem E;
     __shared__ unsigned long long s_lkey[32];
@@ -436,10 +444,16 @@
     __shared__ int s_ncand, s_cnt, s_nonempty;
     __shared__ float s_bv[LE_NW];
     __shared__ int s_bp[LE_NW];
+    __shared__ int s_sc[SPLIT ? LE_SCAP : 1], s_sp[SPLIT ? LE_SCAP : 1], s_sl[SPLIT ? LE_SCAP : 1];
+    __shared__ float s_sh[SPLIT ? LE_SCAP : 1];
+    __shared__ short s_tc[SPLIT ? LE_MAXS * LE_GPS : 1];
+    __shared__ unsigned long long s_lfull[SPLIT ? 32 : 1];
+    __shared__ int s_ns, s_ntc;
     const int tid = threadIdx.x, lane = tid & 63, wave = tid >> 6;
     const int row = blockIdx.x;
-    if (tid < 32) s_lkey[tid] = 0ull;
-    if (tid == 0) { s_ncand = 0; s_cnt = 0; s_nonempty = 0; s_t = -INFINITY; }
+    const int ldz = SPLIT ? 2 * D : D;
+    if (tid < 32) { s_lkey[tid] = 0ull; if (SPLIT) s_lfull[tid] = 0ull; }
+    if (tid == 0) { s_ncand = 0; s_cnt = 0; s_nonempty = 0; s_t = -INFINITY; s_ns = 0; s_ntc = 0; }
     {
         const int s0 = tid, s1 = tid + LE_NT;
         const int c0s = min(s0, S - 1), c1s = min(s1, S - 1);
@@ -513,50 +527,105 @@
         }
     }
     __syncthreads();
-    if (wave == LE_NW - 1) {
+    const int fo = (SPLIT && wave == LE_NW - 1 && lane < n_levels) ? filler_pos[lane] : -1;
+    auto finish_levels = [&](const unsigned long long *lkey) {
         const int l = lane;
         Best b = {-INFINITY, 0x7fffffff};
         if (l < n_levels) {
-            b = best_of_key(l < 32 ? s_lkey[l] : 0ull);
-            out_level[(int64_t)row * n_levels + l] = train_cols[level_winner(b, filler_pos[l], n_train)];
+            b = best_of_key(l < 32 ? lkey[l] : 0ull);
+            out_level[(int64_t)row * n_levels + l] = train_cols[level_winner(b, SPLIT ? fo : filler_pos[l], n_train)];
         }
         const Best top = wave_best(b);
         if (lane == 0 && out_top1) out_top1[row] = top.p < n_train ? train_cols[top.p] : -1;
-    }
-    if (!want_k) return;
+    };
+    if (!SPLIT && wave == LE_NW - 1) finish_levels(s_lkey);
+    if (!SPLIT && !want_k) return;
     if (HGR_LAB_ON(dbg == 2)) return;
-    const float t = s_t;
-    for (int q = tid; q < S * LE_GPS; q += LE_NT) {
+    float t = s_t, t2 = t, delta = 0.f;
+    if (SPLIT) {
+        float nf2 = 0.f;
+        for (int i = lane; i < D; i += 64) { const float x = (float)s_feat[i]; nf2 = fmaf(x, x, nf2); }
+#pragma unroll
+        for (int o = 32; o > 0; o >>= 1) nf2 += __shfl_xor(nf2, o);
+        delta = sqrtf(nf2) * 1.0009765625f * dcoef;
+        t2 = lowered(t, 2.f * delta);
+        t = lowered(t, delta);
+        for (int l = wave; l < n_levels; l += LE_NW) {
+            const unsigned long long lk = s_lkey[l];
+            if (!lk) continue;
+            const float b2 = lowered(best_of_key(lk).v, 2.f * delta);
+            for (int s = level_first[l] + lane; s < level_first[l + 1]; s += 64) {
+                const unsigned long long x = s_keys[s];
+                if (!x) continue;
+                const Best b = best_of_key(x);
+                if (!(b.v >= b2)) continue;
+                int slot = LE_SCAP;
+                if (!(__int_as_float(s_p1[s * LE_GPS + 1]) >= b2)) slot = atomicAdd(&s_ns, 1);
+                if (slot < LE_SCAP) {
+                    s_sc[slot] = s * 32 + ((s_p1[s * LE_GPS] >> 8) & 31); s_sh[slot] = b.v; s_sp[slot] = b.p; s_sl[slot] = l;
+                } else {
+                    const int at = atomicAdd(&s_ntc, 2);
+                    s_tc[at] = (short)(s * LE_GPS); s_tc[at + 1] = (short)(s * LE_GPS + 1);
+                }
+            }
+        }
+    }
+    for (int q = tid; want_k && q < S * LE_GPS; q += LE_NT) {
         const float m1 = s_gm[q];
-        if (m1 > -INFINITY && m1 >= t) {
-            if (s_m2[q] >= t) s_cand[atomicAdd(&s_ncand, 1)] = (short)q;
-            else {
-                const int slot = atomicAdd(&s_cnt, 1);
+        if (m1 > -INFINITY && m1 >= t2) {
+            int slot = LE_SCAP;
+            if (s_m2[q] >= t2) s_cand[atomicAdd(&s_ncand, 1)] = (short)q;
+            else if (!SPLIT) {
+                slot = atomicAdd(&s_cnt, 1);
                 if (slot < LE_CAP) { s_cv[slot] = m1; s_cp[slot] = s_p1[q]; }
-            }
+            } else if ((slot = atomicAdd(&s_ns, 1)) < LE_SCAP) {
+                s_sc[slot] = q * 16 + ((s_p1[(q >> 1) * LE_GPS] >> ((q & 1) * 16)) & 15); s_sh[slot] = m1; s_sl[slot] = -1;
+            } else s_cand[atomicAdd(&s_ncand, 1)] = (short)q;
         }
     }
     __syncthreads();
     int ncand = s_ncand;
     if (HGR_LAB_ON(dbg == 3)) return;
     const int r16 = lane & 15, g = lane >> 4;
-    const int ks = D >> 5;
-    auto scan = [&](auto visit) {
-        for (int ci = wave * 2; ci < ncand; ci += 2 * LE_NW) {
-            const int q0 = s_cand[ci], q1 = s_cand[min(ci + 1, ncand - 1)];
-            const E *w0 = (const E *)zslp + ((int64_t)q0 * 16 + r16) * D + g * 8;
-            const E *w1 = (const E *)zslp + ((int64_t)q1 * 16 + r16) * D + g * 8;
+    const int ks = D >> 5, ksz = ldz >> 5;
+    auto scan_list = [&](const short *list, int n, auto visit) {
+        if constexpr (SPLIT) {
+            for (int ci = LE_NW - 1 - wave; ci < n; ci += LE_NW) {
+                const int q0 = list[ci];
+                const E *w0 = (const E *)zslp + ((int64_t)q0 * 16 + r16) * ldz + g * 8;
+                f32x4 a0 = (f32x4){0.f, 0.f, 0.f, 0.f};
+                for (int kk = 0; kk < ksz; kk += 16) {
+                    vec8 f0[16];
+#pragma unroll
+                    for (int u = 0; u < 16; ++u) f0[u] = *(const vec8 *)(w0 + min(kk + u, ksz - 1) * 32);
+#pragma unroll
+                    for (int u = 0; u < 16; ++u) {
+                        if (kk + u < ksz) {
+                            const int kf = kk + u >= ks ? kk + u - ks : kk + u;
+                            a0 = T16<DT>::mfma16(f0[u], *(const vec8 *)(s_feat + kf * 32 + g * 8), a0);
+                        }
+                    }
+                }
+                const float v0 = (r16 == 0 ? a0[0] : r16 == 1 ? a0[1] : r16 == 2 ? a0[2] : a0[3]) + 0.0f;
+                if (r16 < 4) visit(v0, q0 * 16 + g * 4 + r16);
+            }
+            return;
+        }
+        for (int ci = wave * 2; ci < n; ci += 2 * LE_NW) {
+            const int q0 = list[ci], q1 = list[min(ci + 1, n - 1)];
+            const E *w0 = (const E *)zslp + ((int64_t)q0 * 16 + r16) * ldz + g * 8;
+            const E *w1 = (const E *)zslp + ((int64_t)q1 * 16 + r16) * ldz + g * 8;
             f32x4 a0 = (f32x4){0.f, 0.f, 0.f, 0.f}, a1 = a0;
-            for (int kk = 0; kk < ks; kk += 8) {
+            for (int kk = 0; kk < ksz; kk += 8) {
                 vec8 f0[8], f1[8];
 #pragma unroll
                 for (int u = 0; u < 8; ++u) {
-                    const int kq = min(kk + u, ks - 1);
+                    const int kq = min(kk + u, ksz - 1);
                     f0[u] = *(const vec8 *)(w0 + kq * 32); f1[u] = *(const vec8 *)(w1 + kq * 32);
                 }
 #pragma unroll
                 for (int u = 0; u < 8; ++u) {
-                    if (kk + u < ks) {
+                    if (kk + u < ksz) {
                         const vec8 xf = *(const vec8 *)(s_feat + (kk + u) * 32 + g * 8);
                         a0 = T16<DT>::mfma16(f0[u], xf, a0);
                         a1 = T16<DT>::mfma16(f1[u], xf, a1);
@@ -567,22 +636,56 @@
             float v1 = r16 == 0 ? a1[0] : r16 == 1 ? a1[1] : r16 == 2 ? a1[2] : a1[3];
             v0 += 0.0f; v1 += 0.0f;
             if (r16 < 4) {
-                const int te0 = epos[q0 * 16 + g * 4 + r16];
-                if (te0 >= 0) visit(v0, te0);
-                if (ci + 1 < ncand) {
-                    const int te1 = epos[q1 * 16 + g * 4 + r16];
-                    if (te1 >= 0) visit(v1, te1);
-                }
+                visit(v0, q0 * 16 + g * 4 + r16);
+                if (ci + 1 < n) visit(v1, q1 * 16 + g * 4 + r16);
             }
         }
     };
-    scan([&](float v, int te) {
+    auto scan = [&](auto visit) {
+        scan_list(s_cand, ncand, [&](float v, int c) { const int te = epos[c]; if (te >= 0) visit(v, te); });
+    };
+    auto push = [&](float v, int te) {
         if (v >= t) {
             const int slot = atomicAdd(&s_cnt, 1);
             if (slot < LE_CAP) { s_cv[slot] = v; s_cp[slot] = te; }
         }
-    });
-    __syncthreads();
+    };
+    if (SPLIT) {
+        const int ns = min(s_ns, LE_SCAP);
+        for (int base = wave * 16; base < ns; base += 16 * LE_NW) {
+            const E *w = (const E *)zslp + (int64_t)s_sc[min(base + r16, ns - 1)] * ldz + D + g * 8;
+            f32x4 a;
+#pragma unroll
+            for (int e = 0; e < 4; ++e) a[e] = s_sh[min(base + g * 4 + e, ns - 1)];
+            const int i = min(base + g * 4 + r16, ns - 1), lvl = s_sl[i];
+            vec8 f[16];
+#pragma unroll
+            for (int u = 0; u < 16; ++u) f[u] = *(const vec8 *)(w + min(u, ks - 1) * 32);
+            const int pos = lvl < 0 ? epos[s_sc[i]] : s_sp[i];
+#pragma unroll
+            for (int u = 0; u < 16; ++u)
+                if (u < ks) a = T16<DT>::mfma16(f[u], *(const vec8 *)(s_feat + u * 32 + g * 8), a);
+            const float v = (r16 == 0 ? a[0] : r16 == 1 ? a[1] : r16 == 2 ? a[2] : a[3]) + 0.0f;
+            if (r16 < 4 && base + g * 4 + r16 < ns) {
+                if (lvl < 0) push(v, pos);
+                else atomicMax(&s_lfull[lvl], key_of(v, pos));
+            }
+        }
+        scan_list(s_tc, s_ntc, [&](float v, int c) {
+            const int tp = tpos[c];
+            if (tp < 0) return;
+            int l = 0;
+            while (l + 1 < n_levels && level_first[l + 1] <= (c >> 5)) ++l;
+            atomicMax(&s_lfull[l], key_of(v, tp));
+        });
+    }
+    if (want_k) scan(push);
+    __syncthreads();
+    if (SPLIT) {
+        if (wave == LE_NW - 1) finish_levels(s_lfull);
+        if (tid == 0 && fallback_rows && (s_ns > LE_SCAP || (want_k && s_cnt > LE_CAP))) atomicAdd(fallback_rows, 1);
+        if (!want_k) return;
+    }
     if (HGR_LAB_ON(dbg == 4)) return;
     const int cnt = s_cnt;
     if (cnt <= LE_CAP) {
@@ -593,7 +696,7 @@
     if (tid == 0) s_ncand = 0;
     __syncthreads();
     for (int q = tid; q < S * LE_GPS; q += LE_NT)
-        if (s_gm[q] > -INFINITY && s_gm[q] >= t) s_cand[atomicAdd(&s_ncand, 1)] = (short)q;
+        if (s_gm[q] > -INFINITY && s_gm[q] >= t2) s_cand[atomicAdd(&s_ncand, 1)] = (short)q;
     __syncthreads();
     ncand = s_ncand;
     Best last = {INFINITY, -1};
@@ -610,13 +713,15 @@
 int hgr_logits_eval_rows_launch(const void *feat, const void *zslp, int D, int S, const unsigned long long *keys, const float *tmax,
                                 const int *gp1, const float *gm2, const int32_t *level_first, int n_levels, const int32_t *filler_pos, const int32_t *train_cols, int n_train,
                                 const int32_t *epos, const int32_t *test_cols, int n_test, int k, int32_t *out_level, int32_t *out_top1,
-                                int32_t *out_topk, int rows, int dtype, void *stream) {
+                                int32_t *out_topk, int rows, int dtype, void *stream, const int32_t *tpos, float dcoef, int *fallback_rows) {
     static int dbg = -1;
     if (dbg < 0) dbg = hgr_lab_env("HGR_LE_DBG");
-    if (dtype == HGR_BF16) hipLaunchKernelGGL((logits_eval_rows<HGR_BF16>), dim3(rows), dim3(LE_NT), 0, (hipStream_t)stream, feat, zslp, D, S, keys, tmax, gp1, gm2, level_first,
-                                              n_levels, filler_pos, train_cols, n_train, epos, test_cols, n_test, k, out_level, out_top1, out_topk, dbg, rows);
-    else hipLaunchKernelGGL((logits_eval_rows<HGR_F16>), dim3(rows), dim3(LE_NT), 0, (hipStream_t)stream, feat, zslp, D, S, keys, tmax, gp1, gm2, level_first,
-                            n_levels, filler_pos, train_cols, n_train, epos, test_cols, n_test, k, out_level, out_top1, out_topk, dbg, rows);
+#define LE_LAUNCH(DT, SPLIT) hipLaunchKernelGGL((logits_eval_rows<DT, SPLIT>), dim3(rows), dim3(LE_NT), 0, (hipStream_t)stream, feat, zslp, D, S, keys, tmax, gp1, gm2, \
+        level_first, n_levels, filler_pos, train_cols, n_train, epos, test_cols, n_test, k, out_level, out_top1, out_topk, tpos ? 0 : dbg, rows, tpos, dcoef, fallback_rows)
+    if (tpos) { if (dtype == HGR_BF16) LE_LAUNCH(HGR_BF16, true); else LE_LAUNCH(HGR_F16, true); }
+    else if (dtype == HGR_BF16) LE_LAUNCH(HGR_BF16, false);
+    else LE_LAUNCH(HGR_F16, false);
+#undef LE_LAUNCH
     HGR_CHECK_LAUNCH("hgr_logits_eval (row stage)");
     return HGR_OK;
 }
diff --git a/hgr-net_amd/model/clip_tree.py b/hgr-net_amd/model/clip_tree.py
--- a/hgr-net_amd/model/clip_tree.py
+++ b/hgr-net_amd/model/clip_tree.py
@@ -18,6 +18,7 @@
 
 TAIL_OVERLAP = os.environ.get("HGR_TAIL_OVERLAP", "1") != "0"
 LOGITS_SPLIT = os.environ.get("HGR_LOGITS_SPLIT", "class")
+LOGITS_PROMOTE = os.environ.get("HGR_LOGITS_PROMOTE", "1") != "0"
 
 
 class _StopHead(Exception):
@@ -285,6 +286,9 @@
         b, n = feats.shape[0], self._zsl16.shape[0]
         f16 = torch.empty(feats.shape, dtype=self._zsl16.dtype, device=feats.device)
         zc = self._eval_class_operand() if mode is None else mode[1].zsl
+        if mode is not None and LOGITS_SPLIT == "class" and LOGITS_PROMOTE and zc.shape[1] == 2 * feats.shape[1]:
+            ops.l2norm_rows(feats, y16=f16)
+            return ops.logits_eval_split(f16, mode[1], mode[2])
         if zc is not None and zc.shape[1] == 2 * feats.shape[1]:
             if LOGITS_SPLIT == "feat":
                 f32 = torch.empty_like(feats)
diff --git a/hgr-net_amd/ops.py b/hgr-net_amd/ops.py
--- a/hgr-net_amd/ops.py
+++ b/hgr-net_amd/ops.py
@@ -453,6 +453,8 @@
         self.zsl = None
         self._src = None
         self._ws = None
+        self.dcoef = None
+        self.fallback_rows = None
 
     MAX_SLICES = 1024
 
@@ -466,6 +468,11 @@
             z = zsl16[self.perm]
             z[~self.valid] = 0
             self.zsl, self._src = z.contiguous(), zsl16
+            self.dcoef = None
+            if zsl16.shape[1] == 2 * self.algo_d:
+                self.dcoef = split_bound_coef(self.zsl, self.algo_d)
+                if self.fallback_rows is None or self.fallback_rows.device != self.zsl.device:
+                    self.fallback_rows = torch.zeros(1, dtype=torch.int32, device=self.zsl.device)
         return self
 
     def workspace(self, rows: int, dev) -> torch.Tensor:
@@ -492,6 +499,36 @@
               _dev(lvl), _dev(top1), _dev(topk), _dev(plan.workspace(rows, dev)), DT_OF[feat16.dtype], _stream())
     da = getattr(plan, "algo_d", d)
     _prof_end(ev, 2.0 * rows * ix.n_nodes * da, 2 * rows * da + 2 * ix.n_nodes * da, "logits_eval" + ("_" + stage if stage else ""))
+    return lvl, top1, topk
+
+
+def split_bound_coef(zsplit: torch.Tensor, d: int) -> float:
+    import numpy as np
+    zh, zl = zsplit[:, :d].double().norm(dim=1), zsplit[:, d:].double().norm(dim=1)
+    c = 1.001 * float(zl.max()) + (d // 32) * 2.0 ** -17 * 1.01 * float((zh + zl).max())
+    return float(np.nextafter(np.float32(c), np.float32(np.inf)))
+
+
+def split_delta(feat16: torch.Tensor, plan: LogitsEvalPlan) -> torch.Tensor:
+    return feat16.float().norm(dim=1) * 1.0009765625 * plan.dcoef
+
+
+def logits_eval_split(feat16: torch.Tensor, plan: LogitsEvalPlan, k: int, stage: str = ""):
+    ix = plan.index
+    assert plan.zsl is not None and plan.dcoef is not None, "LogitsEvalPlan.bind(zsl_split16, algo_d) first"
+    assert feat16.is_contiguous() and feat16.dtype == plan.zsl.dtype and 2 * feat16.shape[1] == plan.zsl.shape[1]
+    rows, d = feat16.shape
+    dev = feat16.device
+    lvl = torch.empty((rows, ix.n_levels), dtype=torch.int32, device=dev)
+    top1 = torch.empty((rows, 1), dtype=torch.int32, device=dev)
+    topk = torch.empty((rows, max(k, 1)), dtype=torch.int32, device=dev)
+    ev = _prof_begin()
+    _lib.call({"": "hgr_logits_eval_split", "tile": "hgr_logits_eval_split_tile_stage", "row": "hgr_logits_eval_split_row_stage"}[stage],
+              _dev(feat16), _dev(plan.zsl), rows, d, plan.n_perm, _dev(plan.tpos), _dev(plan.epos), _dev(plan.level_first),
+              ix.n_levels, _dev(ix.filler), _dev(ix.train_cols), ix.n_train, _dev(ix.test_cols), ix.n_test, k,
+              _dev(lvl), _dev(top1), _dev(topk), _dev(plan.workspace(rows, dev)), DT_OF[feat16.dtype], _stream(),
+              plan.dcoef, _dev(plan.fallback_rows))
+    _prof_end(ev, 2.0 * rows * ix.n_nodes * d, 2 * rows * d + 4 * ix.n_nodes * d, "logits_eval" + ("_" + stage if stage else ""))
     return lvl, top1, topk
 
 
diff --git a/include/hgr.h b/include/hgr.h
--- a/include/hgr.h
+++ b/include/hgr.h
@@ -317,6 +317,24 @@
                     int n_levels, const int32_t *filler_pos, const int32_t *train_cols, int n_train,
                     const int32_t *test_cols, int n_test, int k,
                     int32_t *out_level, int32_t *out_top1, int32_t *out_topk, void *workspace, int dtype, void *stream);
+int hgr_logits_eval_split(const void *feat16, const void *zsl_split16, int rows, int D, int n_perm,
+                    const int32_t *tpos_perm, const int32_t *epos_perm, const int32_t *level_first,
+                    int n_levels, const int32_t *filler_pos, const int32_t *train_cols, int n_train,
+                    const int32_t *test_cols, int n_test, int k,
+                    int32_t *out_level, int32_t *out_top1, int32_t *out_topk, void *workspace, int dtype, void *stream,
+                    float dcoef, int32_t *fallback_rows);
+int hgr_logits_eval_split_tile_stage(const void *feat16, const void *zsl_split16, int rows, int D, int n_perm,
+                    const int32_t *tpos_perm, const int32_t *epos_perm, const int32_t *level_first,
+                    int n_levels, const int32_t *filler_pos, const int32_t *train_cols, int n_train,
+                    const int32_t *test_cols, int n_test, int k,
+                    int32_t *out_level, int32_t *out_top1, int32_t *out_topk, void *workspace, int dtype, void *stream,
+                    float dcoef, int32_t *fallback_rows);
+int hgr_logits_eval_split_row_stage(const void *feat16, const void *zsl_split16, int rows, int D, int n_perm,
+                    const int32_t *tpos_perm, const int32_t *epos_perm, const int32_t *level_first,
+                    int n_levels, const int32_t *filler_pos, const int32_t *train_cols, int n_train,
+                    const int32_t *test_cols, int n_test, int k,
+                    int32_t *out_level, int32_t *out_top1, int32_t *out_topk, void *workspace, int dtype, void *stream,
+                    float dcoef, int32_t *fallback_rows);
 
 #define HGR_COMM_ID_BYTES 128
 typedef enum { HGR_COMM_F32 = 0, HGR_COMM_F64 = 1, HGR_COMM_F16 = 2, HGR_COMM_BF16 = 3, HGR_COMM_I32 = 4, HGR_COMM_I64 = 5, HGR_COMM_U8 = 6 } hgr_comm_dtype_t;
```
